# ana-kuznetsova/Policy-Gradient-ASR

Hardware: AMD Instinct MI355X
Metric: utterances/sec (B=32,T=1000,F=80) policy-grad step, 1/2/4/8 MI355X (higher is better)
Workload: dtype f32 (fp32-faithful: fp32 storage and accumulate; every big product -- recurrent sweeps, W_ih projections, input and weight gradients -- on the bf16 MFMA as SIX terms of a 3-plane split hi/mid/lo, every term down to 2^-24 of the product; the small products on the exact fp32 MFMA; the faster bf16x3 mo

## Files before the change

### include/pgasr_hip.h

```cpp
#ifndef PGASR_HIP_H
#define PGASR_HIP_H

#include <stddef.h>
#include <stdint.h>

#ifdef __cplusplus
extern "C" {
#endif

typedef enum pgasr_status {
    PGASR_OK = 0,
    PGASR_ERR_INVALID_ARG = 1,
    PGASR_ERR_LAUNCH = 2,
    PGASR_ERR_WORKSPACE = 3,
    PGASR_ERR_UNSUPPORTED = 4,
    PGASR_ERR_TIMEOUT = 5
} pgasr_status;

#define PGASR_ABI_VERSION 7

int pgasr_abi_version(void);
const char* pgasr_status_string(int status);

size_t pgasr_ctc_workspace_bytes(int T, int B, int V, int Lmax);
int pgasr_ctc_loss_grad(const float* log_probs, const int32_t* targets,
                        const int32_t* input_lengths, const int32_t* target_lengths,
                        int T, int B, int V, int Lmax, int blank,
                        const float* utt_scale, const float* pg_coef, const int32_t* pg_path,
                        float* nll, float* grad_logits,
                        void* workspace, size_t workspace_bytes, void* stream);

int pgasr_ctc_grad_from_lattice(const float* log_probs, const int32_t* input_lengths,
                                const int32_t* target_lengths, int T, int B, int V, int Lmax, int blank,
                                const float* utt_scale, const float* pg_coef, const int32_t* pg_path,
                                int pg_coef_per_frame, float* grad_logits, void* workspace, size_t workspace_bytes,
                                void* stream);

int pgasr_pg_rewards(const int32_t* dist, const int32_t* target_lengths, int B, float lam,
                     float inv_global_batch, float* R_greedy, float* R_sample, float* pg_coef,
                     float* utt_scale, void* stream);
int pgasr_pg_loss_value(const float* log_probs, const int32_t* path, const int32_t* input_lengths,
                        const float* nll, const float* utt_scale, const float* pg_coef,
                        int T, int B, int V, int pg_coef_per_frame, float* terms, void* stream);
int pgasr_pg_step_coefs(const int32_t* paths, const int32_t* input_lengths, const int32_t* prefix_dist, int prefix_stride,
                        const int32_t* token_lengths, const int32_t* target_lengths, int T, int B, int blank,
                        float lam, float inv_global_batch, float* coef, void* stream);

#define PGASR_MAX_SAMPLES 16
#define PGASR_BASELINE_HYPOTHESIS 0
#define PGASR_BASELINE_LEAVE_ONE_OUT 1
int pgasr_frame_sample_multi(const float* scores, int T, int B, int V, int K,
                             uint64_t seed, uint32_t offset, int ctr_stride, int ctr_base,
                             int32_t* greedy_path, int32_t* sample_paths, void* stream);
int pgasr_ctc_grad_from_lattice_multi(const float* log_probs, const int32_t* input_lengths,
                                      const int32_t* target_lengths, int T, int B, int V, int Lmax, int blank,
                                      const float* utt_scale, int K, const float* pg_coef, const int32_t* pg_paths,
                                      float* grad_logits, void* workspace, size_t workspace_bytes, void* stream);
int pgasr_pg_rewards_multi(const int32_t* dist, const int32_t* target_lengths, int B, int K, int baseline,
                           float lam, float inv_global_batch, float* R_baseline, float* R_sample, float* pg_coef,
                           float* utt_scale, void* stream);
int pgasr_pg_loss_value_multi(const float* log_probs, const int32_t* paths, int K, const int32_t* input_lengths,
                              const float* nll, const float* utt_scale, const float* pg_coef,
                              int T, int B, int V, float* terms, void* stream);

#define PGASR_WORD_MAX_STRIDE 4094
int pgasr_word_ids(const int32_t* ref, const int32_t* ref_len, int ref_stride,
                   const int32_t* hyp, const int32_t* hyp_len, int hyp_stride, int N, int delimiter,
                   int32_t* ref_ids, int32_t* ref_words, int32_t* hyp_ids, int32_t* hyp_words, void* stream);
int pgasr_pg_rewards_multi_ex(const int32_t* dist, const int32_t* reward_lengths, const int32_t* target_lengths, int B, int K,
                              int baseline, float lam, float inv_global_batch, float* R_baseline, float* R_sample,
                              float* pg_coef, float* utt_scale, void* stream);

int pgasr_head_logsoftmax(const float* x, long long rows, int K, int ldx, const float* W, const float* bias, int V,
                          float* logits, float* log_probs, void* stream);

int pgasr_frame_argmax_sample(const float* scores, int T, int B, int V,
                              uint64_t seed, uint32_t offset, int ctr_stride, int ctr_base,
                              int32_t* greedy_path, int32_t* sample_path, void* stream);

int pgasr_batch_prep(const float* fmask, int B, int T, const long long* tmask, const long long* targets, int L,
                     int32_t* in_len, int32_t* tg_len, int32_t* targets32, void* stream);
int pgasr_ctc_collapse(const int32_t* paths, const int32_t* lengths, int P, int T, int B,
                       int blank, int32_t* tokens, int32_t* token_lengths, void* stream);

int pgasr_edit_distance(const int32_t* ref, const int32_t* ref_len, int ref_stride,
                        const int32_t* hyp, const int32_t* hyp_len, int hyp_stride,
                        int N, int32_t* dist, int32_t* prefix_dist, void* stream);

int pgasr_reinforce_grad(const float* scores, const int32_t* path, const float* coef,
                         const int32_t* lengths, int T, int B, int V, int accumulate,
                         float* grad, void* stream);

size_t pgasr_gemm_workspace_bytes(int M, int N, int batch, int splitk, int sum_batches);
int pgasr_gemm_f32(int transA, int transB, int M, int N, int K, float alpha,
                   const float* A, int lda, long long strideA,
                   const float* B, int ldb, long long strideB,
                   float* C, int ldc, long long strideC,
                   int batch, int sum_batches, int splitk,
                   const float* bias, const float* bias2, int act, float slope, int accumulate,
                   const float* dact_y, int norm_operand, const float* shift, const float* scale,
                   int precision, const unsigned* xcc_busy, void* workspace, size_t workspace_bytes, void* stream);

int pgasr_split_bf16_planes(const float* src, int rows, int cols, int ld, int transpose,
                            unsigned short* hi, unsigned short* lo, void* stream);
int pgasr_gemm_x3w_f32(int M, int N, int K, const float* A, int lda, const unsigned short* Whi,
                       const unsigned short* Wlo, float* C, int ldc, const float* bias,
                       const float* dact_y, float slope, void* stream);
size_t pgasr_gemm_x3w_feed_workspace_bytes(void);
int pgasr_gemm_x3w_feed_col_tiles(int N);
int pgasr_gemm_x3w_feed_head_items(int N, int K, int groups);
int pgasr_gemm_x3w_feed_f32(int M, int N, int K, const float* A, int lda, const unsigned short* Whi,
                            const unsigned short* Wlo, float* C, int ldc, const float* bias,
                            const unsigned* xcc_busy, unsigned* tiles_done, int order, int phase, int head_groups,
                            void* workspace, size_t workspace_bytes, void* stream);

size_t pgasr_lstm_wgrads_workspace_bytes(int T, int in_dim);
int pgasr_lstm_wgrads_streamed(const float* dgates, const float* x, const float* out, int T, int B, int in_dim,
                               float* dwih_perm, float* dwhh_perm, const unsigned* xcc_busy,
                               const unsigned* slab_done, int* err_word, int planes,
                               void* workspace, size_t workspace_bytes, void* stream);

int pgasr_pack_x6w_planes(const float* src, int rows, int cols, int ld, int transpose, void* pack, void* stream);
int pgasr_split_bf16_planes3(const float* src, int rows, int cols, int ld, int transpose,
                             unsigned short* hi, unsigned short* mid, unsigned short* lo, void* stream);
int pgasr_gemm_x6w_f32(int M, int N, int K, const float* A, int lda, const unsigned short* Whi,
                       const unsigned short* Wmid, const unsigned short* Wlo, float* C, int ldc, const float* bias,
                       const float* dact_y, float slope, void* stream);
size_t pgasr_gemm_x6w_feed_workspace_bytes(void);
int pgasr_gemm_x6w_feed_col_tiles(int N);
int pgasr_gemm_x6w_feed_f32(int M, int N, int K, const float* A, int lda, const unsigned short* Whi,
                            const unsigned short* Wmid, const unsigned short* Wlo, float* C, int ldc, const float* bias,
                            const unsigned* xcc_busy, unsigned* tiles_done, int order,
                            void* workspace, size_t workspace_bytes, void* stream);
int pgasr_gemm_x6w_feed_head_items(int M, int N, int K);
int pgasr_gemm_x6w_feed_phase_f32(int M, int N, int K, const float* A, int lda, const unsigned short* Whi,
                                  const unsigned short* Wmid, const unsigned short* Wlo, float* C, int ldc, const float* bias,
                                  const unsigned* xcc_busy, unsigned* tiles_done, int order, int phase, unsigned* ctrl,
                                  void* workspace, size_t workspace_bytes, void* stream);

int pgasr_attention_ctx(const float* dec, const float* enc, int NQ, int B, int T, int H, float* ctx, void* stream);

int pgasr_lstm_cell_f32(const float* gh, const float* xp, float* c, float* h, float* h_out, int B, int H, void* stream);

size_t pgasr_colsum_workspace_bytes(int rows, int cols);
int pgasr_colsum_f32(const float* X, int rows, int cols, int ld, float* out, float* out2, int accumulate,
                     void* workspace, size_t workspace_bytes, void* stream);

int pgasr_instnorm_stats(const float* x, int B, int F, int T, float eps, float* mean, float* rstd,
                         void* stream);

int pgasr_log_softmax_rows(const float* logits, long long rows, int V, float* log_probs, void* stream);

size_t pgasr_lstm_pack_bytes(int which, int planes);
int pgasr_lstm_pack_weights(const float* w_ih_f, const float* w_hh_f, const float* b_ih_f, const float* b_hh_f,
                            const float* w_ih_r, const float* w_hh_r, const float* b_ih_r, const float* b_hh_r,
                            int in_dim, float* wih_perm, float* bias_perm,
                            void* whh_pack_fwd, void* whh_pack_bwd, int planes, void* stream);
int pgasr_lstm_unpack_grads(const float* dwih_perm, const float* dbias_perm, const float* dwhh_perm, int in_dim,
                            float* dw_ih_f, float* dw_hh_f, float* db_ih_f, float* db_hh_f,
                            float* dw_ih_r, float* dw_hh_r, float* db_ih_r, float* db_hh_r,
                            int accumulate, void* stream);
size_t pgasr_lstm_workspace_bytes(int T, int B, int backward);
int pgasr_lstm_error_offset(int B, int backward, size_t* offset);
int pgasr_lstm_status(const void* workspace, size_t workspace_bytes, int B, int backward, void* stream);
int pgasr_error_flag(const int32_t* word0, const int32_t* word1, float* out, void* stream);
int pgasr_lstm_busy_offset(int B, int backward, size_t* offset);
int pgasr_stream_gate(const unsigned* words, int count, int timeout_us, void* stream);
int pgasr_stream_gate_sum(const unsigned* words, int count, int need, const unsigned* running, int timeout_us, void* stream);
int pgasr_stream_gate_report(const unsigned* words, int count, int need, const unsigned* running, int timeout_us,
                             unsigned* report, void* stream);
int pgasr_stream_probe(unsigned* words, int timeout_us, void* stream);
int pgasr_lstm_layer_fwd(float* gates, float* out, float* cbuf, const void* whh_pack_fwd,
                         const int32_t* lengths, int T, int B, int flags,
                         float* out_drop, float drop_p, uint64_t drop_seed, uint32_t drop_offset,
                         void* workspace, size_t workspace_bytes, void* stream);
int pgasr_lstm_layer_fwd_fed(float* gates, float* out, float* cbuf, const void* whh_pack_fwd,
                             const int32_t* lengths, int T, int B, int flags, const unsigned* fed, int fed_need,
                             float* out_drop, float drop_p, uint64_t drop_seed, uint32_t drop_offset,
                             void* workspace, size_t workspace_bytes, void* stream);
int pgasr_lstm_fed_ok(int T, int B, int flags);
int pgasr_lstm_layer_bwd_fed(float* gates, const float* out, const float* cbuf, const float* dout,
                             const void* whh_pack_bwd, const int32_t* lengths, int T, int B, int flags,
                             float* dbias_part, const unsigned* fed, int fed_need, float drop_p, uint64_t drop_seed,
                             uint32_t drop_offset, void* workspace, size_t workspace_bytes, void* stream);
int pgasr_lstm_layer_bwd(float* gates, const float* out, const float* cbuf, const float* dout,
                         const void* whh_pack_bwd, const int32_t* lengths, int T, int B, int flags,
                         float* dbias_part, void* workspace, size_t workspace_bytes, void* stream);
int pgasr_lstm_wgrad_slabs(int T, int* edges, int max_edges);
int pgasr_lstm_layer_bwd_streamed(float* gates, const float* out, const float* cbuf, const float* dout,
                                  const void* whh_pack_bwd, const int32_t* lengths, int T, int B, int flags,
                                  float* dbias_part, const unsigned* fed, int fed_need, float drop_p, uint64_t drop_seed,
                                  uint32_t drop_offset, unsigned* slab_done,
                                  void* workspace, size_t workspace_bytes, void* stream);

size_t pgasr_beam_workspace_bytes(int T, int B, int V, int beam);
int pgasr_ctc_beam_search(const void* log_probs, int is_f64, long long stride_t, long long stride_b,
                          const int32_t* lengths, int T, int B, int V, int beam, int blank, int flags,
                          int32_t* out_tokens, int32_t* out_len, double* out_score,
                          void* workspace, size_t workspace_bytes, void* stream);

int pgasr_dropout(const float* x, float* y, unsigned long long n, float p, uint64_t seed, uint32_t offset,
                  const float* dact_y, float slope, void* stream);
int pgasr_stream_copy(const void* src, void* dst, unsigned long long bytes, int workgroups, void* stream);
int pgasr_adam_step(float* param, const float* grad, float* exp_avg, float* exp_avg_sq, unsigned long long n,
                    int step, float lr, float beta1, float beta2, float eps, float weight_decay,
                    const int32_t* guard0, const int32_t* guard1, int32_t* applied, void* stream);
#define PGASR_CLIP_STATE_BYTES 32
size_t pgasr_grad_norm_ws_bytes(unsigned long long n);
int pgasr_grad_norm_clip(const float* grad, unsigned long long n, float max_norm, void* ws, size_t ws_bytes,
                         void* state, void* stream);
int pgasr_adam_step_clipped(float* param, const float* grad, float* exp_avg, float* exp_avg_sq, unsigned long long n,
                            int step, float lr, float beta1, float beta2, float eps, float weight_decay,
                            const int32_t* guard0, const int32_t* guard1, int32_t* applied, const void* clip_state,
                            void* stream);

int pgasr_feat_frames(const float* wave, const int32_t* n_samples, const int32_t* n_frames, int B,
                      long long wave_stride, int Tmax, float* frames, void* stream);
int pgasr_feat_power(const float* spec, long long rows, float* power, void* stream);
int pgasr_feat_db(float* mel, const int32_t* n_frames, int B, int Tmax, int n_mels, float top_db, void* stream);
int pgasr_feat_deltas_stack(const float* mfcc, const int32_t* n_frames, int B, int Tmax, int n_mfcc,
                            float* feat, float* fmask, void* stream);
int pgasr_feat_stack(const float* x, const int32_t* n_frames, int B, int Tmax, int C, float* feat, float* fmask, void* stream);

#ifdef __cplusplus
}
#endif
#endif
```

### policy_gradient_asr_amd/_lib.py

```python
import ctypes as C
import os

import torch

_HERE = os.path.dirname(os.path.abspath(__file__))
LIB_PATH = os.environ.get("PGASR_HIP_LIB", os.path.join(_HERE, "libpgasr_hip.so"))

c_f32p = C.c_void_p
c_i32p = C.c_void_p
c_ptr = C.c_void_p

SIGNATURES = {
    "pgasr_abi_version": (C.c_int, []),
    "pgasr_status_string": (C.c_char_p, [C.c_int]),
    "pgasr_ctc_workspace_bytes": (C.c_size_t, [C.c_int, C.c_int, C.c_int, C.c_int]),
    "pgasr_ctc_loss_grad": (C.c_int, [c_f32p, c_i32p, c_i32p, c_i32p, C.c_int, C.c_int, C.c_int, C.c_int,
                                      C.c_int, c_f32p, c_f32p, c_i32p, c_f32p, c_f32p, c_ptr, C.c_size_t, c_ptr]),
    "pgasr_ctc_grad_from_lattice": (C.c_int, [c_f32p, c_i32p, c_i32p, C.c_int, C.c_int, C.c_int, C.c_int, C.c_int,
                                              c_f32p, c_f32p, c_i32p, C.c_int, c_f32p, c_ptr, C.c_size_t, c_ptr]),
    "pgasr_pg_rewards": (C.c_int, [c_i32p, c_i32p, C.c_int, C.c_float, C.c_float, c_f32p, c_f32p, c_f32p, c_f32p, c_ptr]),
    "pgasr_pg_loss_value": (C.c_int, [c_f32p, c_i32p, c_i32p, c_f32p, c_f32p, c_f32p, C.c_int, C.c_int, C.c_int, C.c_int,
                                      c_f32p, c_ptr]),
    "pgasr_head_logsoftmax": (C.c_int, [c_f32p, C.c_longlong, C.c_int, C.c_int, c_f32p, c_f32p, C.c_int, c_f32p, c_f32p, c_ptr]),
    "pgasr_pg_step_coefs": (C.c_int, [c_i32p, c_i32p, c_i32p, C.c_int, c_i32p, c_i32p, C.c_int, C.c_int, C.c_int,
                                      C.c_float, C.c_float, c_f32p, c_ptr]),
    "pgasr_frame_argmax_sample": (C.c_int, [c_f32p, C.c_int, C.c_int, C.c_int, C.c_uint64, C.c_uint32, C.c_int, C.c_int,
                                            c_i32p, c_i32p, c_ptr]),
    "pgasr_frame_sample_multi": (C.c_int, [c_f32p, C.c_int, C.c_int, C.c_int, C.c_int, C.c_uint64, C.c_uint32, C.c_int, C.c_int,
                                           c_i32p, c_i32p, c_ptr]),
    "pgasr_ctc_grad_from_lattice_multi": (C.c_int, [c_f32p, c_i32p, c_i32p, C.c_int, C.c_int, C.c_int, C.c_int, C.c_int,
                                                    c_f32p, C.c_int, c_f32p, c_i32p, c_f32p, c_ptr, C.c_size_t, c_ptr]),
    "pgasr_pg_rewards_multi": (C.c_int, [c_i32p, c_i32p, C.c_int, C.c_int, C.c_int, C.c_float, C.c_float, c_f32p, c_f32p, c_f32p,
                                         c_f32p, c_ptr]),
    "pgasr_pg_loss_value_multi": (C.c_int, [c_f32p, c_i32p, C.c_int, c_i32p, c_f32p, c_f32p, c_f32p, C.c_int, C.c_int, C.c_int,
                                            c_f32p, c_ptr]),
    "pgasr_word_ids": (C.c_int, [c_i32p, c_i32p, C.c_int, c_i32p, c_i32p, C.c_int, C.c_int, C.c_int, c_i32p, c_i32p, c_i32p, c_i32p,
                                 c_ptr]),
    "pgasr_pg_rewards_multi_ex": (C.c_int, [c_i32p, c_i32p, c_i32p, C.c_int, C.c_int, C.c_int, C.c_float, C.c_float, c_f32p, c_f32p,
                                            c_f32p, c_f32p, c_ptr]),
    "pgasr_batch_prep": (C.c_int, [c_f32p, C.c_int, C.c_int, c_ptr, c_ptr, C.c_int, c_i32p, c_i32p, c_i32p, c_ptr]),
    "pgasr_ctc_collapse": (C.c_int, [c_i32p, c_i32p, C.c_int, C.c_int, C.c_int, C.c_int, c_i32p, c_i32p, c_ptr]),
    "pgasr_edit_distance": (C.c_int, [c_i32p, c_i32p, C.c_int, c_i32p, c_i32p, C.c_int, C.c_int,
                                      c_i32p, c_i32p, c_ptr]),
    "pgasr_reinforce_grad": (C.c_int, [c_f32p, c_i32p, c_f32p, c_i32p, C.c_int, C.c_int, C.c_int, C.c_int,
                                       c_f32p, c_ptr]),
    "pgasr_beam_workspace_bytes": (C.c_size_t, [C.c_int] * 4),
    "pgasr_ctc_beam_search": (C.c_int, [c_ptr, C.c_int, C.c_longlong, C.c_longlong, c_i32p, C.c_int, C.c_int, C.c_int,
                                        C.c_int, C.c_int, C.c_int, c_i32p, c_i32p, c_ptr, c_ptr, C.c_size_t, c_ptr]),
    "pgasr_dropout": (C.c_int, [c_f32p, c_f32p, C.c_ulonglong, C.c_float, C.c_uint64, C.c_uint32, c_f32p, C.c_float, c_ptr]),
    "pgasr_stream_copy": (C.c_int, [c_ptr, c_ptr, C.c_ulonglong, C.c_int, c_ptr]),
    "pgasr_adam_step": (C.c_int, [c_f32p, c_f32p, c_f32p, c_f32p, C.c_ulonglong, C.c_int, C.c_float, C.c_float,
                                  C.c_float, C.c_float, C.c_float, c_i32p, c_i32p, c_i32p, c_ptr]),
    "pgasr_adam_step_clipped": (C.c_int, [c_f32p, c_f32p, c_f32p, c_f32p, C.c_ulonglong, C.c_int, C.c_float, C.c_float,
                                          C.c_float, C.c_float, C.c_float, c_i32p, c_i32p, c_i32p, c_ptr, c_ptr]),
    "pgasr_grad_norm_ws_bytes": (C.c_size_t, [C.c_ulonglong]),
    "pgasr_grad_norm_clip": (C.c_int, [c_f32p, C.c_ulonglong, C.c_float, c_ptr, C.c_size_t, c_ptr, c_ptr]),
    "pgasr_gemm_workspace_bytes": (C.c_size_t, [C.c_int] * 5),
    "pgasr_gemm_f32": (C.c_int, [C.c_int, C.c_int, C.c_int, C.c_int, C.c_int, C.c_float,
                                 c_f32p, C.c_int, C.c_longlong, c_f32p, C.c_int, C.c_longlong,
                                 c_f32p, C.c_int, C.c_longlong, C.c_int, C.c_int, C.c_int,
                                 c_f32p, c_f32p, C.c_int, C.c_float, C.c_int,
                                 c_f32p, C.c_int, c_f32p, c_f32p, C.c_int, c_ptr, c_ptr, C.c_size_t, c_ptr]),
    "pgasr_split_bf16_planes": (C.c_int, [c_f32p, C.c_int, C.c_int, C.c_int, C.c_int, c_ptr, c_ptr, c_ptr]),
    "pgasr_gemm_x3w_f32": (C.c_int, [C.c_int, C.c_int, C.c_int, c_f32p, C.c_int, c_ptr, c_ptr, c_f32p, C.c_int,
                                     c_f32p, c_f32p, C.c_float, c_ptr]),
    "pgasr_gemm_x3w_feed_workspace_bytes": (C.c_size_t, []),
    "pgasr_gemm_x3w_feed_col_tiles": (C.c_int, [C.c_int]),
    "pgasr_gemm_x3w_feed_head_items": (C.c_int, [C.c_int, C.c_int, C.c_int]),
    "pgasr_gemm_x3w_feed_f32": (C.c_int, [C.c_int, C.c_int, C.c_int, c_f32p, C.c_int, c_ptr, c_ptr, c_f32p, C.c_int,
                                          c_f32p, c_ptr, c_ptr, C.c_int, C.c_int, C.c_int, c_ptr, C.c_size_t, c_ptr]),
    "pgasr_feat_frames": (C.c_int, [c_f32p, c_i32p, c_i32p, C.c_int, C.c_longlong, C.c_int, c_f32p, c_ptr]),
    "pgasr_feat_power": (C.c_int, [c_f32p, C.c_longlong, c_f32p, c_ptr]),
    "pgasr_feat_db": (C.c_int, [c_f32p, c_i32p, C.c_int, C.c_int, C.c_int, C.c_float, c_ptr]),
    "pgasr_feat_deltas_stack": (C.c_int, [c_f32p, c_i32p, C.c_int, C.c_int, C.c_int, c_f32p, c_f32p, c_ptr]),
    "pgasr_feat_stack": (C.c_int, [c_f32p, c_i32p, C.c_int, C.c_int, C.c_int, c_f32p, c_f32p, c_ptr]),
    "pgasr_colsum_workspace_bytes": (C.c_size_t, [C.c_int, C.c_int]),
    "pgasr_colsum_f32": (C.c_int, [c_f32p, C.c_int, C.c_int, C.c_int, c_f32p, c_f32p, C.c_int,
                                   c_ptr, C.c_size_t, c_ptr]),
    "pgasr_instnorm_stats": (C.c_int, [c_f32p, C.c_int, C.c_int, C.c_int, C.c_float, c_f32p, c_f32p, c_ptr]),
    "pgasr_log_softmax_rows": (C.c_int, [c_f32p, C.c_longlong, C.c_int, c_f32p, c_ptr]),
    "pgasr_lstm_pack_bytes": (C.c_size_t, [C.c_int, C.c_int]),
    "pgasr_lstm_pack_weights": (C.c_int, [c_f32p] * 8 + [C.c_int, c_f32p, c_f32p, c_ptr, c_ptr, C.c_int, c_ptr]),
    "pgasr_lstm_unpack_grads": (C.c_int, [c_f32p, c_f32p, c_f32p, C.c_int] + [c_f32p] * 8 + [C.c_int, c_ptr]),
    "pgasr_lstm_workspace_bytes": (C.c_size_t, [C.c_int, C.c_int, C.c_int]),
    "pgasr_lstm_error_offset": (C.c_int, [C.c_int, C.c_int, C.POINTER(C.c_size_t)]),
    "pgasr_lstm_busy_offset": (C.c_int, [C.c_int, C.c_int, C.POINTER(C.c_size_t)]),
    "pgasr_lstm_status": (C.c_int, [c_ptr, C.c_size_t, C.c_int, C.c_int, c_ptr]),
    "pgasr_stream_gate": (C.c_int, [c_ptr, C.c_int, C.c_int, c_ptr]),
    "pgasr_stream_gate_sum": (C.c_int, [c_ptr, C.c_int, C.c_int, c_ptr, C.c_int, c_ptr]),
    "pgasr_stream_gate_report": (C.c_int, [c_ptr, C.c_int, C.c_int, c_ptr, C.c_int, c_ptr, c_ptr]),
    "pgasr_stream_probe": (C.c_int, [c_ptr, C.c_int, c_ptr]),
    "pgasr_lstm_layer_fwd": (C.c_int, [c_f32p, c_f32p, c_f32p, c_ptr, c_i32p, C.c_int, C.c_int, C.c_int,
                                       c_f32p, C.c_float, C.c_uint64, C.c_uint32, c_ptr, C.c_size_t, c_ptr]),
    "pgasr_lstm_layer_fwd_fed": (C.c_int, [c_f32p, c_f32p, c_f32p, c_ptr, c_i32p, C.c_int, C.c_int, C.c_int, c_ptr, C.c_int,
                                           c_f32p, C.c_float, C.c_uint64, C.c_uint32, c_ptr, C.c_size_t, c_ptr]),
    "pgasr_lstm_fed_ok": (C.c_int, [C.c_int, C.c_int, C.c_int]),
    "pgasr_lstm_layer_bwd_fed": (C.c_int, [c_f32p, c_f32p, c_f32p, c_f32p, c_ptr, c_i32p, C.c_int, C.c_int, C.c_int,
                                           c_f32p, c_ptr, C.c_int, C.c_float, C.c_uint64, C.c_uint32, c_ptr, C.c_size_t, c_ptr]),
    "pgasr_lstm_layer_bwd": (C.c_int, [c_f32p, c_f32p, c_f32p, c_f32p, c_ptr, c_i32p, C.c_int, C.c_int, C.c_int,
                                       c_f32p, c_ptr, C.c_size_t, c_ptr]),
    "pgasr_lstm_wgrad_slabs": (C.c_int, [C.c_int, c_i32p, C.c_int]),
    "pgasr_lstm_layer_bwd_streamed": (C.c_int, [c_f32p, c_f32p, c_f32p, c_f32p, c_ptr, c_i32p, C.c_int, C.c_int, C.c_int,
                                                c_f32p, c_ptr, C.c_int, C.c_float, C.c_uint64, C.c_uint32, c_ptr,
                                                c_ptr, C.c_size_t, c_ptr]),
    "pgasr_lstm_wgrads_workspace_bytes": (C.c_size_t, [C.c_int, C.c_int]),
    "pgasr_lstm_wgrads_streamed": (C.c_int, [c_f32p, c_f32p, c_f32p, C.c_int, C.c_int, C.c_int, c_f32p, c_f32p, c_ptr,
                                             c_ptr, c_ptr, C.c_int, c_ptr, C.c_size_t, c_ptr]),
    "pgasr_error_flag": (C.c_int, [c_i32p, c_i32p, c_f32p, c_ptr]),
    "pgasr_attention_ctx": (C.c_int, [c_f32p, c_f32p, C.c_int, C.c_int, C.c_int, C.c_int, c_f32p, c_ptr]),
    "pgasr_lstm_cell_f32": (C.c_int, [c_f32p, c_f32p, c_f32p, c_f32p, c_f32p, C.c_int, C.c_int, c_ptr]),
    "pgasr_pack_x6w_planes": (C.c_int, [c_f32p, C.c_int, C.c_int, C.c_int, C.c_int, c_ptr, c_ptr]),
    "pgasr_split_bf16_planes3": (C.c_int, [c_f32p, C.c_int, C.c_int, C.c_int, C.c_int, c_ptr, c_ptr, c_ptr, c_ptr]),
    "pgasr_gemm_x6w_f32": (C.c_int, [C.c_int, C.c_int, C.c_int, c_f32p, C.c_int, c_ptr, c_ptr, c_ptr, c_f32p, C.c_int,
                                     c_f32p, c_f32p, C.c_float, c_ptr]),
    "pgasr_gemm_x6w_feed_workspace_bytes": (C.c_size_t, []),
    "pgasr_gemm_x6w_feed_col_tiles": (C.c_int, [C.c_int]),
    "pgasr_gemm_x6w_feed_f32": (C.c_int, [C.c_int, C.c_int, C.c_int, c_f32p, C.c_int, c_ptr, c_ptr, c_ptr, c_f32p, C.c_int,
                                          c_f32p, c_ptr, c_ptr, C.c_int, c_ptr, C.c_size_t, c_ptr]),
    "pgasr_gemm_x6w_feed_head_items": (C.c_int, [C.c_int, C.c_int, C.c_int]),
    "pgasr_gemm_x6w_feed_phase_f32": (C.c_int, [C.c_int, C.c_int, C.c_int, c_f32p, C.c_int, c_ptr, c_ptr, c_ptr, c_f32p, C.c_int,
                                                c_f32p, c_ptr, c_ptr, C.c_int, C.c_int, c_ptr, c_ptr, C.c_size_t, c_ptr]),
}


class PgasrError(RuntimeError):
    pass


TIMEOUT = 5


_lib = None


def load():
    global _lib
    if _lib is not None:
        return _lib
    if not os.path.exists(LIB_PATH):
        raise PgasrError(
            f"{LIB_PATH} is missing: build it with `python -c 'import __graft_entry__ as g; g.build()'` "
            "or `make -C policy_gradient_asr_amd/csrc`.  There is no CPU fallback.")
    lib = C.CDLL(LIB_PATH)
    for name, (res, args) in SIGNATURES.items():
        fn = getattr(lib, name)
        fn.restype = res
        fn.argtypes = args
    if lib.pgasr_abi_version() != 7:
        raise PgasrError("libpgasr_hip.so ABI version mismatch")
    _lib = lib
    return lib


def check(status, what):
    if status != 0:
        msg = load().pgasr_status_string(status).decode()
        raise PgasrError(f"{what} failed: status {status} ({msg})")
```

### policy_gradient_asr_amd/csrc/common.h

```cpp
#pragma once
#include <hip/hip_runtime.h>
#include <stdint.h>
#include <math.h>
#include <stdio.h>
#include <stdlib.h>
#include "pgasr_hip.h"

#define PGASR_WAVE 64

#define PGASR_LAUNCH_KERNEL(...)                               \
    do {                                                       \
        (void)hipGetLastError();                               \
        hipLaunchKernelGGL(__VA_ARGS__);                       \
    } while (0)

#define PGASR_CHECK_LAUNCH()                                                                  \
    do {                                                                                      \
        hipError_t e__ = hipGetLastError();                                                   \
        if (e__ != hipSuccess) {                                                              \
            if (getenv("PGASR_DEBUG"))                                                        \
                fprintf(stderr, "[pgasr] %s:%d launch failed: %s\n", __FILE__, __LINE__,      \
                        hipGetErrorString(e__));                                              \
            return PGASR_ERR_LAUNCH;                                                          \
        }                                                                                     \
    } while (0)

static inline size_t pgasr_align_up(size_t x, size_t a) { return (x + a - 1) / a * a; }

#define PGASR_NEG_INF (-INFINITY)

__device__ __forceinline__ float wave_sum(float v) {
#pragma unroll
    for (int o = 32; o > 0; o >>= 1) v += __shfl_xor(v, o, 64);
    return v;
}
__device__ __forceinline__ float wave_max(float v) {
#pragma unroll
    for (int o = 32; o > 0; o >>= 1) v = fmaxf(v, __shfl_xor(v, o, 64));
    return v;
}

__device__ __forceinline__ void philox4x32_10(uint32_t c0, uint32_t c1, uint32_t c2, uint32_t c3,
                                              uint32_t k0, uint32_t k1, uint32_t out[4]) {
#pragma unroll
    for (int r = 0; r < 10; ++r) {
        const uint64_t p0 = (uint64_t)0xD2511F53u * c0;
        const uint64_t p1 = (uint64_t)0xCD9E8D57u * c2;
        const uint32_t n0 = (uint32_t)(p1 >> 32) ^ c1 ^ k0;
        const uint32_t n1 = (uint32_t)p1;
        const uint32_t n2 = (uint32_t)(p0 >> 32) ^ c3 ^ k1;
        const uint32_t n3 = (uint32_t)p0;
        c0 = n0; c1 = n1; c2 = n2; c3 = n3;
        k0 += 0x9E3779B9u; k1 += 0xBB67AE85u;
    }
    out[0] = c0; out[1] = c1; out[2] = c2; out[3] = c3;
}

#ifndef PGASR_WSLAB_NUM
#define PGASR_WSLAB_NUM 5
#define PGASR_WSLAB_DEN 4
#define PGASR_WSLAB_CAP 128
#endif
__host__ __device__ inline int pgasr_wslab_next(int s) { const int n = ((s * PGASR_WSLAB_NUM) / PGASR_WSLAB_DEN + 4) & ~7; return n > PGASR_WSLAB_CAP ? PGASR_WSLAB_CAP : n; }
__host__ __device__ inline int pgasr_wslab_count(int T) {
    int h = 0, s = 16, n = 1;
    while (T - h > s + s / 2) { h += s; s = pgasr_wslab_next(s); ++n; }
    return n;
}
__host__ __device__ inline int pgasr_wslab_edge(int T, int i) {
    int h = 0, s = 16;
    for (int j = 0; j < i; ++j) {
        if (T - h <= s + s / 2) return T;
        h += s; s = pgasr_wslab_next(s);
    }
    return h;
}

struct PgasrTn256Args {
    const float* A; const float* B; float* partial;
    int M, N, K, lda, ldb;
    long long sA, sB;
    int batch, splitk, kper;
    float alpha;
    unsigned* queue;
    const unsigned* xcc_busy;
    int diag;
    const unsigned* gate;
    const float* gate_base;
    int gate_T, gate_B, gate_nbg;
    int tslabs;
    int* gate_err;
};
bool pgasr_internal_tn256_ok(const PgasrTn256Args& a, int tk = 32);
int pgasr_internal_tn256_launch(PgasrTn256Args a, int masked_then_unmasked, hipStream_t st, const PgasrTn256Args* second = nullptr);
int pgasr_internal_tn6_launch(PgasrTn256Args a, int masked_then_unmasked, hipStream_t st, const PgasrTn256Args* second = nullptr);

struct PgasrX3cArgs {
    const float* A; const unsigned short* Whi; const unsigned short* Wlo; float* C;
    int M, N, K, lda, ldc;
    const float* bias; const float* dact_y; float slope;
    int feed;
    unsigned* queue; const unsigned* xcc_busy; unsigned* tiles_done;
    int mt_count, nt_count, order, quarters, split_tiles;
    float* slabs; unsigned* arrive;
};
size_t pgasr_internal_x3c_slab_bytes();
int pgasr_internal_x3c_launch(const PgasrX3cArgs& a, hipStream_t st);
```

### policy_gradient_asr_amd/csrc/gemm.hip

```cpp
#include "common.h"

namespace {

constexpr int BM = 128, BN = 128, BK = 16, PADF = 4;
constexpr int GEMM_THREADS = 256;

typedef __attribute__((ext_vector_type(16))) float f32x16;

struct GemmArgs {
    const float* A; const float* B; float* C;
    int M, N, K, lda, ldb, ldc;
    long long sA, sB, sC;
    int batch, splitk, kper;
    float alpha;
    const float* bias; const float* bias2;
    int act; float slope;
    int accumulate;
    const float* dact_y;
    int norm_operand;
    const float* shift; const float* scale;
    float* partial;
    unsigned* queue;
    const unsigned* xcc_busy;
    int tx, ty, tz;
    int wide;
};

__device__ __forceinline__ void store_tiles_fast(const GemmArgs& g, const f32x16 (&acc)[2][2], int m0, int n0, int wm, int wn,
                                                 int lane, int z, int bidx, bool live) {
    const int cl = lane & 31, rq = lane >> 5;
    if (g.partial) {
        float* slab = g.partial + (size_t)z * g.M * g.N;
        __amdgpu_buffer_rsrc_t prs = __builtin_amdgcn_make_buffer_rsrc(slab, 0, (int)(unsigned)((size_t)g.M * g.N * 4), 0x00020000);
#pragma unroll
        for (int i = 0; i < 2; ++i)
#pragma unroll
            for (int j = 0; j < 2; ++j) {
                const int n = n0 + wn * 64 + j * 32 + cl;
                const bool ok = live && n < g.N;
                const unsigned o0 = (unsigned)(((size_t)(m0 + wm * 64 + i * 32 + 4 * rq) * g.N + n) * 4);
#pragma unroll
                for (int r = 0; r < 16; ++r)
                    __builtin_amdgcn_raw_buffer_store_b32(__float_as_uint(g.alpha * acc[i][j][r]), prs,
                                                          ok ? o0 + (unsigned)(((r & 3) + 8 * (r >> 2)) * g.N * 4) : 0xFFFFFFFFu, 0, 0);
            }
        return;
    }
    float* Cb = g.C + (size_t)bidx * g.sC;
    const unsigned cbytes = (unsigned)(((size_t)(g.M - 1) * g.ldc + g.N) * 4);
    __amdgpu_buffer_rsrc_t crs = __builtin_amdgcn_make_buffer_rsrc(Cb, 0, (int)cbytes, 0x00020000);
    __amdgpu_buffer_rsrc_t yrs = __builtin_amdgcn_make_buffer_rsrc(const_cast<float*>(g.dact_y ? g.dact_y + (size_t)bidx * g.sC : Cb), 0, (int)cbytes, 0x00020000);
    float bsum[2];
#pragma unroll
    for (int j = 0; j < 2; ++j) {
        const int n = n0 + wn * 64 + j * 32 + cl;
        bsum[j] = 0.f;
        if (n < g.N) {
            if (g.bias) bsum[j] += g.bias[n];
            if (g.bias2) bsum[j] += g.bias2[n];
        }
    }
    const bool lk = g.act == 1;
    if (!g.dact_y && !g.accumulate) {
#pragma unroll
        for (int i = 0; i < 2; ++i)
#pragma unroll
            for (int j = 0; j < 2; ++j) {
                const int n = n0 + wn * 64 + j * 32 + cl;
                const bool ok = live && n < g.N;
                const unsigned o0 = (unsigned)(((size_t)(m0 + wm * 64 + i * 32 + 4 * rq) * g.ldc + n) * 4);
#pragma unroll
                for (int r = 0; r < 16; ++r) {
                    float v = g.alpha * acc[i][j][r] + bsum[j];
                    v = (lk && !(v > 0.f)) ? v * g.slope : v;
                    __builtin_amdgcn_raw_buffer_store_b32(__float_as_uint(v), crs, ok ? o0 + (unsigned)(((r & 3) + 8 * (r >> 2)) * g.ldc * 4) : 0xFFFFFFFFu, 0, 0);
                }
            }
        return;
    }
    const bool hd = g.dact_y != nullptr, ha = g.accumulate != 0;
#pragma unroll
    for (int i = 0; i < 2; ++i)
#pragma unroll
        for (int j = 0; j < 2; ++j) {
            const int n = n0 + wn * 64 + j * 32 + cl;
            const bool ok = live && n < g.N;
            const unsigned o0 = (unsigned)(((size_t)(m0 + wm * 64 + i * 32 + 4 * rq) * g.ldc + n) * 4);
            float f[16], c0[16];
#pragma unroll
            for (int r = 0; r < 16; ++r) {
                const unsigned o = ok ? o0 + (unsigned)(((r & 3) + 8 * (r >> 2)) * g.ldc * 4) : 0xFFFFFFFFu;
                f[r] = hd ? (__uint_as_float(__builtin_amdgcn_raw_buffer_load_b32(yrs, o, 0, 0)) > 0.f ? 1.f : g.slope) : 1.f;
                c0[r] = ha ? __uint_as_float(__builtin_amdgcn_raw_buffer_load_b32(crs, o, 0, 0)) : 0.f;
            }
#pragma unroll
            for (int r = 0; r < 16; ++r) {
                const unsigned o = ok ? o0 + (unsigned)(((r & 3) + 8 * (r >> 2)) * g.ldc * 4) : 0xFFFFFFFFu;
                float v = g.alpha * acc[i][j][r] + bsum[j];
                v = (lk && !(v > 0.f)) ? v * g.slope : v;
                v = v * f[r] + c0[r];
                __builtin_amdgcn_raw_buffer_store_b32(__float_as_uint(v), crs, o, 0, 0);
            }
        }
}

template <bool KCONTIG>
__device__ __forceinline__ void load_strip(const float* __restrict__ P, int ld, int mn_base, int mn_lim,
                                           int k_base, int k_lim, int tid, bool vec_ok, float v[8]) {
    if (KCONTIG) {
        const int mn = mn_base + (tid >> 1);
        const int k0 = k_base + (tid & 1) * 8;
        if (mn < mn_lim && k0 + 8 <= k_lim && vec_ok) {
            const float4* p = reinterpret_cast<const float4*>(P + (size_t)mn * ld + k0);
            const float4 a = p[0], b = p[1];
            v[0] = a.x; v[1] = a.y; v[2] = a.z; v[3] = a.w; v[4] = b.x; v[5] = b.y; v[6] = b.z; v[7] = b.w;
        } else {
#pragma unroll
            for (int i = 0; i < 8; ++i)
                v[i] = (mn < mn_lim && k0 + i < k_lim) ? P[(size_t)mn * ld + k0 + i] : 0.f;
        }
    } else {
        const int k = k_base + (tid >> 4);
        const int mn0 = mn_base + (tid & 15) * 8;
        if (k < k_lim && mn0 + 8 <= mn_lim && vec_ok) {
            const float4* p = reinterpret_cast<const float4*>(P + (size_t)k * ld + mn0);
            const float4 a = p[0], b = p[1];
            v[0] = a.x; v[1] = a.y; v[2] = a.z; v[3] = a.w; v[4] = b.x; v[5] = b.y; v[6] = b.z; v[7] = b.w;
        } else {
#pragma unroll
            for (int i = 0; i < 8; ++i)
                v[i] = (k < k_lim && mn0 + i < mn_lim) ? P[(size_t)k * ld + mn0 + i] : 0.f;
        }
    }
}

template <bool KCONTIG>
__device__ __forceinline__ void store_strip(float (*S)[BM + PADF], int tid, const float v[8]) {
    if (KCONTIG) {
        const int mn = tid >> 1, k0 = (tid & 1) * 8;
#pragma unroll
        for (int i = 0; i < 8; ++i) S[k0 + i][mn] = v[i];
    } else {
        const int k = tid >> 4, mn0 = (tid & 15) * 8;
        *reinterpret_cast<float4*>(&S[k][mn0]) = make_float4(v[0], v[1], v[2], v[3]);
        *reinterpret_cast<float4*>(&S[k][mn0 + 4]) = make_float4(v[4], v[5], v[6], v[7]);
    }
}

__device__ __forceinline__ void swizzled_tile(int& bx, int& by, int& bz) {
    const unsigned gx = gridDim.x, gy = gridDim.y, gz = gridDim.z;
    const unsigned nwg = gx * gy * gz;
    const unsigned L = blockIdx.x + gx * (blockIdx.y + gy * blockIdx.z);
    const unsigned q = nwg / 8, r = nwg % 8;
    const unsigned xcd = L % 8, i = L / 8;
    const unsigned t = (xcd < r ? xcd * (q + 1) : r * (q + 1) + (xcd - r) * q) + i;
    bx = (int)(t % gx); by = (int)((t / gx) % gy); bz = (int)(t / (gx * gy));
}

template <bool TA, bool TB>
__global__ __launch_bounds__(GEMM_THREADS) void gemm_f32_kernel(GemmArgs g) {
    __shared__ __attribute__((aligned(16))) float As[2][BK][BM + PADF];
    __shared__ __attribute__((aligned(16))) float Bs[2][BK][BN + PADF];
    const int tid = threadIdx.x, lane = tid & 63, wid = tid >> 6;
    const int wm = wid >> 1, wn = wid & 1;
    int tbx, tby, z;
    swizzled_tile(tbx, tby, z);
    const int bidx = z / g.splitk, sidx = z % g.splitk;
    const int m0 = tby * BM, n0 = tbx * BN;
    const float* A = g.A + (size_t)bidx * g.sA;
    const float* B = g.B + (size_t)bidx * g.sB;
    const int kbeg = sidx * g.kper;
    const int kend = min(g.K, kbeg + g.kper);
    const bool vecA = ((g.lda & 3) == 0) && ((((size_t)A) & 15) == 0);
    const bool vecB = ((g.ldb & 3) == 0) && ((((size_t)B) & 15) == 0);
    float nsh = 0.f, nsc = 1.f;
    if (g.norm_operand) { nsh = g.shift[bidx]; nsc = g.scale[bidx]; }

    f32x16 acc[2][2];
#pragma unroll
    for (int i = 0; i < 2; ++i)
#pragma unroll
        for (int j = 0; j < 2; ++j)
#pragma unroll
            for (int r = 0; r < 16; ++r) acc[i][j][r] = 0.f;

    float ra[8], rb[8];
    auto gload = [&](int kb) {
        load_strip<!TA>(A, g.lda, m0, g.M, kb, kend, tid, vecA, ra);
        load_strip<TB>(B, g.ldb, n0, g.N, kb, kend, tid, vecB, rb);
        if (g.norm_operand == 1) {
#pragma unroll
            for (int i = 0; i < 8; ++i) ra[i] = (ra[i] - nsh) * nsc;
        } else if (g.norm_operand == 2) {
#pragma unroll
            for (int i = 0; i < 8; ++i) rb[i] = (rb[i] - nsh) * nsc;
        }
    };
    auto fix_edges = [&](int kb) {
        if (g.norm_operand == 1) {
            if (!TA) { const int mn = m0 + (tid >> 1), k0 = kb + (tid & 1) * 8;
#pragma unroll
                for (int i = 0; i < 8; ++i) if (!(mn < g.M && k0 + i < kend)) ra[i] = 0.f; }
            else { const int k = kb + (tid >> 4), mn0 = m0 + (tid & 15) * 8;
#pragma unroll
                for (int i = 0; i < 8; ++i) if (!(k < kend && mn0 + i < g.M)) ra[i] = 0.f; }
        } else if (g.norm_operand == 2) {
            if (TB) { const int mn = n0 + (tid >> 1), k0 = kb + (tid & 1) * 8;
#pragma unroll
                for (int i = 0; i < 8; ++i) if (!(mn < g.N && k0 + i < kend)) rb[i] = 0.f; }
            else { const int k = kb + (tid >> 4), mn0 = n0 + (tid & 15) * 8;
#pragma unroll
                for (int i = 0; i < 8; ++i) if (!(k < kend && mn0 + i < g.N)) rb[i] = 0.f; }
        }
    };

    if (kbeg < kend) {
        gload(kbeg); fix_edges(kbeg);
        store_strip<!TA>(As[0], tid, ra);
        store_strip<TB>(Bs[0], tid, rb);
    }
    __syncthreads();
    int cur = 0;
    for (int kb = kbeg; kb < kend; kb += BK) {
        const bool more = kb + BK < kend;
        if (more) { gload(kb + BK); fix_edges(kb + BK); }
        const int r = lane & 31, kh = lane >> 5;
#pragma unroll
        for (int kk = 0; kk < BK; kk += 2) {
            const float a0 = As[cur][kk + kh][wm * 64 + r];
            const float a1 = As[cur][kk + kh][wm * 64 + 32 + r];
            const float b0 = Bs[cur][kk + kh][wn * 64 + r];
            const float b1 = Bs[cur][kk + kh][wn * 64 + 32 + r];
            acc[0][0] = __builtin_amdgcn_mfma_f32_32x32x2f32(a0, b0, acc[0][0], 0, 0, 0);
            acc[0][1] = __builtin_amdgcn_mfma_f32_32x32x2f32(a0, b1, acc[0][1], 0, 0, 0);
            acc[1][0] = __builtin_amdgcn_mfma_f32_32x32x2f32(a1, b0, acc[1][0], 0, 0, 0);
            acc[1][1] = __builtin_amdgcn_mfma_f32_32x32x2f32(a1, b1, acc[1][1], 0, 0, 0);
        }
        if (more) {
            store_strip<!TA>(As[cur ^ 1], tid, ra);
            store_strip<TB>(Bs[cur ^ 1], tid, rb);
        }
        __syncthreads();
        cur ^= 1;
    }

    if (!g.wide) { store_tiles_fast(g, acc, m0, n0, wm, wn, lane, z, bidx, true); return; }
    const int cl = lane & 31, rq = lane >> 5;
#pragma unroll
    for (int i = 0; i < 2; ++i)
#pragma unroll
        for (int j = 0; j < 2; ++j) {
            const int n = n0 + wn * 64 + j * 32 + cl;
            if (n >= g.N) continue;
            float bsum = 0.f;
            if (!g.partial) {
                if (g.bias) bsum += g.bias[n];
                if (g.bias2) bsum += g.bias2[n];
            }
#pragma unroll
            for (int r = 0; r < 16; ++r) {
                const int m = m0 + wm * 64 + i * 32 + (r & 3) + 8 * (r >> 2) + 4 * rq;
                if (m >= g.M) continue;
                float v = g.alpha * acc[i][j][r];
                if (g.partial) {
                    g.partial[((size_t)z * g.M + m) * g.N + n] = v;
                } else {
                    float* c = g.C + (size_t)bidx * g.sC + (size_t)m * g.ldc + n;
                    v += bsum;
                    if (g.act == 1) v = v > 0.f ? v : v * g.slope;
                    if (g.dact_y) v *= (g.dact_y[(size_t)bidx * g.sC + (size_t)m * g.ldc + n] > 0.f ? 1.f : g.slope);
                    if (g.accumulate) v += *c;
                    *c = v;
                }
            }
        }
}

constexpr int XBK = 32, XPITCH = 40;

typedef __attribute__((ext_vector_type(8))) __bf16 bf16x8_t;
typedef __attribute__((ext_vector_type(4))) unsigned u32x4_t;

__device__ __forceinline__ void split2(float x0, float x1, unsigned& hi_pk, unsigned& lo_pk) {
    typedef __attribute__((ext_vector_type(2))) __bf16 bf2;
    typedef __attribute__((ext_vector_type(2))) float f2;
    const bf2 h = __builtin_convertvector((f2){x0, x1}, bf2);
    hi_pk = __builtin_bit_cast(unsigned, h);
    const float h0 = __uint_as_float(hi_pk << 16), h1 = __uint_as_float(hi_pk & 0xFFFF0000u);
    const bf2 l = __builtin_convertvector((f2){x0 - h0, x1 - h1}, bf2);
    lo_pk = __builtin_bit_cast(unsigned, l);
}

__device__ __forceinline__ void xload_strip(const float* __restrict__ P, int ld, int mn_base, int mn_lim,
                                            int k_base, int k_lim, int tid, bool vec_ok, float v[16]) {
    const int mn = mn_base + (tid >> 1);
    const int k0 = k_base + (tid & 1) * 16;
    if (mn < mn_lim && k0 + 16 <= k_lim && vec_ok) {
        const float4* p = reinterpret_cast<const float4*>(P + (size_t)mn * ld + k0);
#pragma unroll
        for (int i = 0; i < 4; ++i) { const float4 a = p[i]; v[4 * i] = a.x; v[4 * i + 1] = a.y; v[4 * i + 2] = a.z; v[4 * i + 3] = a.w; }
    } else {
#pragma unroll
        for (int i = 0; i < 16; ++i) v[i] = (mn < mn_lim && k0 + i < k_lim) ? P[(size_t)mn * ld + k0 + i] : 0.f;
    }
}

__device__ __forceinline__ void xstore_strip(unsigned short* hi, unsigned short* lo, int tid, const float v[16]) {
    const int row = tid >> 1, k0 = (tid & 1) * 16;
    unsigned h[8], l[8];
#pragma unroll
    for (int i = 0; i < 8; ++i) split2(v[2 * i], v[2 * i + 1], h[i], l[i]);
    u32x4_t* ph = reinterpret_cast<u32x4_t*>(hi + row * XPITCH + k0);
    u32x4_t* pl = reinterpret_cast<u32x4_t*>(lo + row * XPITCH + k0);
    ph[0] = (u32x4_t){h[0], h[1], h[2], h[3]}; ph[1] = (u32x4_t){h[4], h[5], h[6], h[7]};
    pl[0] = (u32x4_t){l[0], l[1], l[2], l[3]}; pl[1] = (u32x4_t){l[4], l[5], l[6], l[7]};
}

constexpr int TPITCH = 160;
static_assert(XBK * TPITCH == BM * XPITCH, "both LDS images fill the same array");
typedef __attribute__((ext_vector_type(4))) short s16x4_t;
typedef __attribute__((ext_vector_type(8))) short s16x8_t;
typedef __attribute__((ext_vector_type(2))) unsigned u32x2_t;

__device__ __forceinline__ void tload_strip(const float* __restrict__ P, int ld, int mn_base, int mn_lim,
                                            int k_base, int k_lim, int tid, bool vec_ok, float v[16]) {
    const int mn0 = mn_base + (tid & 31) * 4;
    if (vec_ok && k_base + XBK <= k_lim && mn_base + BM <= mn_lim) {
        const float* p = P + (size_t)(k_base + (tid >> 5)) * ld + mn0;
#pragma unroll
        for (int i = 0; i < 4; ++i) {
            const float4 a = *reinterpret_cast<const float4*>(p + (size_t)(8 * i) * ld);
            v[4 * i] = a.x; v[4 * i + 1] = a.y; v[4 * i + 2] = a.z; v[4 * i + 3] = a.w;
        }
        return;
    }
#pragma unroll
    for (int i = 0; i < 4; ++i) {
        const int k = k_base + (tid >> 5) + 8 * i;
#pragma unroll
        for (int c = 0; c < 4; ++c) v[4 * i + c] = (k < k_lim && mn0 + c < mn_lim) ? P[(size_t)k * ld + mn0 + c] : 0.f;
    }
}

__device__ __forceinline__ void tstore_strip(unsigned short* hi, unsigned short* lo, int tid, const float v[16]) {
#pragma unroll
    for (int i = 0; i < 4; ++i) {
        unsigned h0, l0, h1, l1;
        split2(v[4 * i], v[4 * i + 1], h0, l0);
        split2(v[4 * i + 2], v[4 * i + 3], h1, l1);
        const int o = ((tid >> 5) + 8 * i) * TPITCH + (tid & 31) * 4;
        *reinterpret_cast<u32x2_t*>(hi + o) = (u32x2_t){h0, h1};
        *reinterpret_cast<u32x2_t*>(lo + o) = (u32x2_t){l0, l1};
    }
}

__device__ __forceinline__ bf16x8_t tr_frag(const unsigned short* p) {
    typedef s16x4_t __attribute__((address_space(3))) * lds_s16x4_ptr;
    const s16x4_t a = __builtin_amdgcn_ds_read_tr16_b64_v4i16((lds_s16x4_ptr)(p));
    const s16x4_t b = __builtin_amdgcn_ds_read_tr16_b64_v4i16((lds_s16x4_ptr)(p + 4 * TPITCH));
    return __builtin_bit_cast(bf16x8_t, (s16x8_t){a.x, a.y, a.z, a.w, b.x, b.y, b.z, b.w});
}

template <bool TA, bool TB, bool QUEUE>
__global__ __launch_bounds__(GEMM_THREADS, 2) void gemm_bf16x3_kernel(GemmArgs g) {
    __shared__ __attribute__((aligned(16))) unsigned short S[2][2][2][BM * XPITCH];
    const int tid = threadIdx.x, lane = tid & 63, wid = tid >> 6;
    const int wm = wid >> 1, wn = wid & 1;
    int tbx = 0, tby = 0, z = 0;
    bool live = true;
    if (QUEUE) {
        const unsigned xcc = __builtin_amdgcn_s_getreg(((4 - 1) << 11) | (0 << 6) | 20) & 0xFu;
        const bool allowed = g.xcc_busy == nullptr ||
                             __hip_atomic_load(g.xcc_busy + (xcc & 7u), __ATOMIC_RELAXED, __HIP_MEMORY_SCOPE_AGENT) == 0u;
        unsigned* mailbox = reinterpret_cast<unsigned*>(&S[0][0][0][0]);
        if (tid == 0) *mailbox = allowed ? __hip_atomic_fetch_add(g.queue, 1u, __ATOMIC_RELAXED, __HIP_MEMORY_SCOPE_AGENT) : 0xFFFFFFFFu;
        __syncthreads();
        const unsigned t = *mailbox;
        __syncthreads();
        live = t < (unsigned)g.tx * g.ty * g.tz;
        if (live) { tbx = (int)(t % g.tx); tby = (int)((t / g.tx) % g.ty); z = (int)(t / ((unsigned)g.tx * g.ty)); }
    } else {
        swizzled_tile(tbx, tby, z);
    }
    const int bidx = z / g.splitk, sidx = z % g.splitk;
    const int m0 = tby * BM, n0 = tbx * BN;
    const float* A = g.A + (size_t)bidx * g.sA;
    const float* B = g.B + (size_t)bidx * g.sB;
    const int kbeg = sidx * g.kper;
    const int kend = live ? min(g.K, kbeg + g.kper) : kbeg;
    const bool vecA = ((g.lda & 3) == 0) && ((((size_t)A) & 15) == 0);
    const bool vecB = ((g.ldb & 3) == 0) && ((((size_t)B) & 15) == 0);

    f32x16 acc[2][2];
#pragma unroll
    for (int i = 0; i < 2; ++i)
#pragma unroll
        for (int j = 0; j < 2; ++j)
#pragma unroll
// ... 125 lines not shown
    if (bias2) v += bias2[n];
    if (act == 1) v = v > 0.f ? v : v * slope;
    float* c = C + (size_t)m * ldc + n;
    if (accumulate) v += *c;
    *c = v;
}

__global__ __launch_bounds__(256) void colsum_partial_kernel(const float* __restrict__ X, int rows, int cols, int ld,
                                                             int rows_per_block, float* __restrict__ partial) {
    __shared__ float red[4][64];
    const int c = blockIdx.x * 64 + (threadIdx.x & 63);
    const int rl = threadIdx.x >> 6;
    const int r0 = blockIdx.y * rows_per_block, r1 = min(rows, r0 + rows_per_block);
    float s = 0.f;
    if (c < cols)
        for (int r = r0 + rl; r < r1; r += 4) s += X[(size_t)r * ld + c];
    red[rl][threadIdx.x & 63] = s;
    __syncthreads();
    if (rl == 0 && c < cols)
        partial[(size_t)blockIdx.y * cols + c] = (red[0][threadIdx.x] + red[1][threadIdx.x]) + (red[2][threadIdx.x] + red[3][threadIdx.x]);
}
__global__ __launch_bounds__(256) void colsum_final_kernel(const float* __restrict__ partial, int nparts, int cols,
                                                           float* __restrict__ out, float* __restrict__ out2, int accumulate) {
    const int c = blockIdx.x * 256 + threadIdx.x;
    if (c >= cols) return;
    float s = 0.f;
    for (int p = 0; p < nparts; ++p) s += partial[(size_t)p * cols + c];
    if (accumulate) { out[c] += s; if (out2) out2[c] += s; }
    else { out[c] = s; if (out2) out2[c] = s; }
}

__global__ __launch_bounds__(1024) void instnorm_stats_kernel(const float* __restrict__ x, long long n_per, float eps,
                                                              float* __restrict__ mean, float* __restrict__ rstd) {
    __shared__ double s1[16], s2[16];
    const float* p = x + (size_t)blockIdx.x * n_per;
    double a = 0.0, b = 0.0;
    long long done = 0;
    if (((n_per & 3) == 0) && ((((size_t)x) & 15) == 0)) {
        const float4* p4 = reinterpret_cast<const float4*>(p);
        const long long n4 = n_per >> 2;
        double a1 = 0.0, b1 = 0.0;
        long long i = threadIdx.x;
        for (; i + 3 * 1024 < n4; i += 4 * 1024) {
            const float4 u0 = p4[i], u1 = p4[i + 1024], u2 = p4[i + 2 * 1024], u3 = p4[i + 3 * 1024];
            a += ((double)u0.x + (double)u0.y) + ((double)u0.z + (double)u0.w);
            b += ((double)u0.x * u0.x + (double)u0.y * u0.y) + ((double)u0.z * u0.z + (double)u0.w * u0.w);
            a1 += ((double)u1.x + (double)u1.y) + ((double)u1.z + (double)u1.w);
            b1 += ((double)u1.x * u1.x + (double)u1.y * u1.y) + ((double)u1.z * u1.z + (double)u1.w * u1.w);
            a += ((double)u2.x + (double)u2.y) + ((double)u2.z + (double)u2.w);
            b += ((double)u2.x * u2.x + (double)u2.y * u2.y) + ((double)u2.z * u2.z + (double)u2.w * u2.w);
            a1 += ((double)u3.x + (double)u3.y) + ((double)u3.z + (double)u3.w);
            b1 += ((double)u3.x * u3.x + (double)u3.y * u3.y) + ((double)u3.z * u3.z + (double)u3.w * u3.w);
        }
        for (; i < n4; i += 1024) {
            const float4 u = p4[i];
            a += ((double)u.x + (double)u.y) + ((double)u.z + (double)u.w);
            b += ((double)u.x * u.x + (double)u.y * u.y) + ((double)u.z * u.z + (double)u.w * u.w);
        }
        a += a1; b += b1;
        done = n_per;
    }
    for (long long i = done + threadIdx.x; i < n_per; i += 1024) { const double v = p[i]; a += v; b += v * v; }
#pragma unroll
    for (int o = 32; o > 0; o >>= 1) { a += __shfl_xor(a, o, 64); b += __shfl_xor(b, o, 64); }
    if ((threadIdx.x & 63) == 0) { s1[threadIdx.x >> 6] = a; s2[threadIdx.x >> 6] = b; }
    __syncthreads();
    if (threadIdx.x == 0) {
        double ta = 0.0, tb = 0.0;
        for (int i = 0; i < 16; ++i) { ta += s1[i]; tb += s2[i]; }
        const double mu = ta / (double)n_per;
        double var = tb / (double)n_per - mu * mu;
        if (var < 0.0) var = 0.0;
        mean[blockIdx.x] = (float)mu;
        rstd[blockIdx.x] = (float)(1.0 / sqrt(var + (double)eps));
    }
}

}

static int gemm_launch(GemmArgs& g, int transA, int transB, int sum_batches, int precision, const unsigned* xcc_busy, void* workspace,
                       size_t workspace_bytes, hipStream_t st) {
    const int Z = g.batch * g.splitk;
    const bool use_partial = (g.splitk > 1) || sum_batches;
    const bool queue_mode = precision >= 1 && xcc_busy != nullptr;
    const size_t head = 256;
    if (use_partial || queue_mode) {
        const size_t need = head + (use_partial ? (size_t)Z * g.M * g.N * sizeof(float) : 0);
        if (!workspace || workspace_bytes < need) return PGASR_ERR_WORKSPACE;
    }
    g.partial = use_partial ? (float*)((char*)workspace + head) : nullptr;
    g.queue = nullptr; g.xcc_busy = nullptr;
    dim3 grid((g.N + BN - 1) / BN, (g.M + BM - 1) / BM, Z);
    if (grid.y > 65535 || grid.z > 65535) return PGASR_ERR_UNSUPPORTED;
    g.tx = (int)grid.x; g.ty = (int)grid.y; g.tz = (int)grid.z;
    if (queue_mode) {
        g.queue = (unsigned*)workspace; g.xcc_busy = xcc_busy;
        if (hipMemsetAsync(workspace, 0, head, st) != hipSuccess) return PGASR_ERR_LAUNCH;
    }
    const unsigned ntiles_q = grid.x * grid.y * grid.z;

    bool done_tn256 = false;
    if (precision >= 1 && transA && !transB && use_partial && g.norm_operand == 0) {
        PgasrTn256Args t{g.A, g.B, g.partial, g.M, g.N, g.K, g.lda, g.ldb, g.sA, g.sB, g.batch, g.splitk, g.kper, g.alpha,
                         queue_mode ? g.queue : nullptr, queue_mode ? g.xcc_busy : nullptr, getenv("PGASR_TN_DIAG") ? atoi(getenv("PGASR_TN_DIAG")) : 0,
                         nullptr, nullptr, 0, 0, 0, 0, nullptr};
        if (pgasr_internal_tn256_ok(t)) {
            const int st_ = precision == 2 ? pgasr_internal_tn6_launch(t, queue_mode ? 1 : 0, st) : pgasr_internal_tn256_launch(t, queue_mode ? 1 : 0, st);
            if (st_ != PGASR_OK) return st_;
            done_tn256 = true;
        }
    }
    if (done_tn256) {
    }
    else if (precision == 2) return PGASR_ERR_UNSUPPORTED;
    else if (precision == 1) {
        if (queue_mode) {
            for (int pass = 0; pass < 2; ++pass) {
                dim3 qgrid(pass == 0 ? 2u * ntiles_q + 8u : ntiles_q);
                if (pass == 1) g.xcc_busy = nullptr;
                if (!transA && !transB) PGASR_LAUNCH_KERNEL((gemm_bf16x3_kernel<false, false, true>), qgrid, dim3(GEMM_THREADS), 0, st, g);
                else if (!transA && transB) PGASR_LAUNCH_KERNEL((gemm_bf16x3_kernel<false, true, true>), qgrid, dim3(GEMM_THREADS), 0, st, g);
                else if (transA && !transB) PGASR_LAUNCH_KERNEL((gemm_bf16x3_kernel<true, false, true>), qgrid, dim3(GEMM_THREADS), 0, st, g);
                else PGASR_LAUNCH_KERNEL((gemm_bf16x3_kernel<true, true, true>), qgrid, dim3(GEMM_THREADS), 0, st, g);
                PGASR_CHECK_LAUNCH();
            }
        }
        else if (!transA && !transB) PGASR_LAUNCH_KERNEL((gemm_bf16x3_kernel<false, false, false>), grid, dim3(GEMM_THREADS), 0, st, g);
        else if (!transA && transB) PGASR_LAUNCH_KERNEL((gemm_bf16x3_kernel<false, true, false>), grid, dim3(GEMM_THREADS), 0, st, g);
        else if (transA && !transB) PGASR_LAUNCH_KERNEL((gemm_bf16x3_kernel<true, false, false>), grid, dim3(GEMM_THREADS), 0, st, g);
        else PGASR_LAUNCH_KERNEL((gemm_bf16x3_kernel<true, true, false>), grid, dim3(GEMM_THREADS), 0, st, g);
    }
    else if (!transA && !transB) PGASR_LAUNCH_KERNEL((gemm_f32_kernel<false, false>), grid, dim3(GEMM_THREADS), 0, st, g);
    else if (!transA && transB) PGASR_LAUNCH_KERNEL((gemm_f32_kernel<false, true>), grid, dim3(GEMM_THREADS), 0, st, g);
    else if (transA && !transB) PGASR_LAUNCH_KERNEL((gemm_f32_kernel<true, false>), grid, dim3(GEMM_THREADS), 0, st, g);
    else PGASR_LAUNCH_KERNEL((gemm_f32_kernel<true, true>), grid, dim3(GEMM_THREADS), 0, st, g);
    PGASR_CHECK_LAUNCH();
    if (use_partial) {
        const size_t total = (size_t)g.M * g.N;
        const int nout = sum_batches ? 1 : g.batch;
        PGASR_LAUNCH_KERNEL(gemm_reduce_kernel, dim3((unsigned)((total + 255) / 256), nout), dim3(256), 0, st,
                           g.partial, Z / nout, g.M, g.N, g.C, g.ldc, g.sC, g.bias, g.bias2, g.act, g.slope,
                           g.accumulate);
        PGASR_CHECK_LAUNCH();
    }
    return PGASR_OK;
}

extern "C" size_t pgasr_gemm_workspace_bytes(int M, int N, int batch, int splitk, int sum_batches) {
    if (M <= 0 || N <= 0 || batch <= 0 || splitk <= 0) return 0;
    if (splitk <= 1 && !sum_batches) return 256;
    return 256 + (size_t)batch * splitk * M * N * sizeof(float);
}

extern "C" int pgasr_gemm_f32(int transA, int transB, int M, int N, int K, float alpha,
                              const float* A, int lda, long long strideA,
                              const float* B, int ldb, long long strideB,
                              float* C, int ldc, long long strideC,
                              int batch, int sum_batches, int splitk,
                              const float* bias, const float* bias2, int act, float slope, int accumulate,
                              const float* dact_y, int norm_operand, const float* shift, const float* scale,
                              int precision, const unsigned* xcc_busy, void* workspace, size_t workspace_bytes, void* stream) {
    if (!A || !B || !C || M <= 0 || N <= 0 || K <= 0 || batch <= 0 || splitk <= 0) return PGASR_ERR_INVALID_ARG;
    if (norm_operand < 0 || norm_operand > 2 || (norm_operand && (!shift || !scale))) return PGASR_ERR_INVALID_ARG;
    if (act < 0 || act > 1 || precision < 0 || precision > 2) return PGASR_ERR_INVALID_ARG;
    if ((splitk > 1 || sum_batches) && dact_y) return PGASR_ERR_INVALID_ARG;
    GemmArgs g;
    g.A = A; g.B = B; g.C = C; g.M = M; g.N = N; g.K = K; g.lda = lda; g.ldb = ldb; g.ldc = ldc;
    g.sA = strideA; g.sB = strideB; g.sC = strideC; g.batch = batch; g.splitk = splitk;
    int kper = (K + splitk - 1) / splitk;
    const int kq = precision >= 1 ? XBK : BK;
    kper = (kper + kq - 1) / kq * kq;
    g.kper = kper;
    g.alpha = alpha; g.bias = bias; g.bias2 = bias2; g.act = act; g.slope = slope; g.accumulate = accumulate;
    g.dact_y = dact_y; g.norm_operand = norm_operand; g.shift = shift; g.scale = scale; g.partial = nullptr;
    g.wide = (((size_t)(M - 1) * ldc + N) * 4 >= ((size_t)1 << 32) || (size_t)M * N * 4 >= ((size_t)1 << 32)) ? 1 : 0;
    return gemm_launch(g, transA, transB, sum_batches, precision, xcc_busy, workspace, workspace_bytes, (hipStream_t)stream);
}

extern "C" int pgasr_lstm_wgrad_slabs(int T, int* edges, int max_edges) {
    if (T <= 0) return 0;
    const int n = pgasr_wslab_count(T);
    for (int i = 0; edges && i <= n && i < max_edges; ++i) edges[i] = pgasr_wslab_edge(T, i);
    return n;
}
extern "C" size_t pgasr_lstm_wgrads_workspace_bytes(int T, int in_dim) {
    if (in_dim <= 0 || T <= 0) return 0;
    return 256 + (size_t)pgasr_wslab_count(T) * ((size_t)2048 * in_dim + (size_t)2 * 1024 * 256) * sizeof(float);
}
extern "C" int pgasr_lstm_wgrads_streamed(const float* dgates, const float* x, const float* out, int T, int B, int in_dim,
                                          float* dwih_perm, float* dwhh_perm, const unsigned* xcc_busy,
                                          const unsigned* slab_done, int* err_word, int planes,
                                          void* workspace, size_t workspace_bytes, void* stream) {
    constexpr int H = 256, G = 2 * 4 * H;
    if (!dgates || !x || !out || !dwih_perm || !dwhh_perm || T <= 1 || B <= 0 || in_dim <= 0) return PGASR_ERR_INVALID_ARG;
    if (planes != 2 && planes != 3) return PGASR_ERR_INVALID_ARG;
    const size_t need = pgasr_lstm_wgrads_workspace_bytes(T, in_dim);
    if (!workspace || workspace_bytes < need) return PGASR_ERR_WORKSPACE;
    hipStream_t st = (hipStream_t)stream;
    const int nslab = pgasr_wslab_count(T);
    float* part_ih = (float*)((char*)workspace + 256);
    float* part_hh = part_ih + (size_t)nslab * G * in_dim;
    const long long K_ih = (long long)T * B, K_hh = (long long)(T - 1) * B;
    if (K_ih >= ((long long)1 << 31)) return PGASR_ERR_UNSUPPORTED;
    PgasrTn256Args ih{dgates, x, part_ih, G, in_dim, (int)K_ih, G, in_dim, 0, 0, 1, nslab, 0, 1.f,
                      (unsigned*)workspace, xcc_busy, 0, slab_done, dgates, T, B, (B + 15) / 16, 1, err_word};
    PgasrTn256Args hh{dgates + (size_t)B * G, out, part_hh, 4 * H, H, (int)K_hh, G, 2 * H, (long long)4 * H - (long long)B * G,
                      (long long)B * 2 * H + H, 2, nslab, 0, 1.f,
                      (unsigned*)workspace, xcc_busy, 0, slab_done, dgates, T, B, (B + 15) / 16, 1, err_word};
    const int tk = planes == 3 ? 16 : 32;
    if (!pgasr_internal_tn256_ok(ih, tk) || !pgasr_internal_tn256_ok(hh, tk)) return PGASR_ERR_UNSUPPORTED;
    if (hipMemsetAsync(workspace, 0, 256, st) != hipSuccess) return PGASR_ERR_LAUNCH;
    const int rc = planes == 3 ? pgasr_internal_tn6_launch(ih, 1, st, &hh) : pgasr_internal_tn256_launch(ih, 1, st, &hh);
    if (rc != PGASR_OK) return rc;
    PGASR_LAUNCH_KERNEL(gemm_reduce_kernel, dim3((unsigned)(((size_t)G * in_dim + 255) / 256), 1), dim3(256), 0, st,
                       part_ih, nslab, G, in_dim, dwih_perm, in_dim, (long long)0, (const float*)nullptr, (const float*)nullptr, 0, 0.f, 0);
    PGASR_CHECK_LAUNCH();
    PGASR_LAUNCH_KERNEL(gemm_reduce_kernel, dim3((unsigned)(((size_t)4 * H * H + 255) / 256), 2), dim3(256), 0, st,
                       part_hh, nslab, 4 * H, H, dwhh_perm, H, (long long)4 * H * H, (const float*)nullptr, (const float*)nullptr, 0, 0.f, 0);
    PGASR_CHECK_LAUNCH();
    return PGASR_OK;
}

extern "C" size_t pgasr_colsum_workspace_bytes(int rows, int cols) {
    if (rows <= 0 || cols <= 0) return 0;
    const int rpb = 512;
    return (size_t)((rows + rpb - 1) / rpb) * cols * sizeof(float);
}

extern "C" int pgasr_colsum_f32(const float* X, int rows, int cols, int ld, float* out, float* out2, int accumulate,
                                void* workspace, size_t workspace_bytes, void* stream) {
    if (!X || !out || rows <= 0 || cols <= 0 || ld < cols) return PGASR_ERR_INVALID_ARG;
    const int rpb = 512;
    const int nparts = (rows + rpb - 1) / rpb;
    if (!workspace || workspace_bytes < (size_t)nparts * cols * sizeof(float)) return PGASR_ERR_WORKSPACE;
    hipStream_t st = (hipStream_t)stream;
    PGASR_LAUNCH_KERNEL(colsum_partial_kernel, dim3((cols + 63) / 64, nparts), dim3(256), 0, st, X, rows, cols, ld, rpb,
                       (float*)workspace);
    PGASR_CHECK_LAUNCH();
    PGASR_LAUNCH_KERNEL(colsum_final_kernel, dim3((cols + 255) / 256), dim3(256), 0, st, (const float*)workspace, nparts,
                       cols, out, out2, accumulate);
    PGASR_CHECK_LAUNCH();
    return PGASR_OK;
}

extern "C" int pgasr_instnorm_stats(const float* x, int B, int F, int T, float eps, float* mean, float* rstd,
                                    void* stream) {
    if (!x || !mean || !rstd || B <= 0 || F <= 0 || T <= 0) return PGASR_ERR_INVALID_ARG;
    PGASR_LAUNCH_KERNEL(instnorm_stats_kernel, dim3(B), dim3(1024), 0, (hipStream_t)stream, x, (long long)F * T, eps,
                       mean, rstd);
    PGASR_CHECK_LAUNCH();
    return PGASR_OK;
}
```

### policy_gradient_asr_amd/csrc/optim.hip

```cpp
#include "common.h"

namespace {

__device__ __forceinline__ void keep4(unsigned long long quad, uint32_t offset, uint32_t k0, uint32_t k1,
                                      uint32_t thresh, bool keep[4]) {
    uint32_t r[4];
    philox4x32_10((uint32_t)quad, (uint32_t)(quad >> 32), offset, 0u, k0, k1, r);
#pragma unroll
    for (int i = 0; i < 4; ++i) keep[i] = r[i] >= thresh;
}

__global__ __launch_bounds__(256) void dropout_kernel(const float* __restrict__ x, float* __restrict__ y,
                                                      unsigned long long n, uint32_t thresh, float scale,
                                                      uint32_t k0, uint32_t k1, uint32_t offset,
                                                      const float* __restrict__ dact_y, float slope) {
    const unsigned long long nq = (n + 3) / 4;
    for (unsigned long long q = (unsigned long long)blockIdx.x * 256 + threadIdx.x; q < nq;
         q += (unsigned long long)gridDim.x * 256) {
        bool keep[4];
        keep4(q, offset, k0, k1, thresh, keep);
        const unsigned long long i = q * 4;
        if (i + 4 <= n) {
            float4 v = *reinterpret_cast<const float4*>(x + i);
            if (dact_y) {
                const float4 a = *reinterpret_cast<const float4*>(dact_y + i);
                v.x *= a.x > 0.f ? 1.f : slope; v.y *= a.y > 0.f ? 1.f : slope;
                v.z *= a.z > 0.f ? 1.f : slope; v.w *= a.w > 0.f ? 1.f : slope;
            }
            float4 o;
            o.x = keep[0] ? v.x * scale : 0.f; o.y = keep[1] ? v.y * scale : 0.f;
            o.z = keep[2] ? v.z * scale : 0.f; o.w = keep[3] ? v.w * scale : 0.f;
            *reinterpret_cast<float4*>(y + i) = o;
        } else {
            for (int k = 0; k < 4 && i + k < n; ++k)
                y[i + k] = keep[k] ? x[i + k] * scale * (dact_y ? (dact_y[i + k] > 0.f ? 1.f : slope) : 1.f) : 0.f;
        }
    }
}

struct ClipState { float norm, scale; int32_t nonfinite, pad, n_clipped, n_nonfinite, pad2[2]; };

template <bool CLIP>
__global__ __launch_bounds__(256) void adam_kernel(float* __restrict__ p, const float* __restrict__ g,
                                                   float* __restrict__ m, float* __restrict__ v, unsigned long long n,
                                                   float lr, float beta1, float beta2, float eps, int call,
                                                   float weight_decay, const int32_t* __restrict__ guard0,
                                                   const int32_t* __restrict__ guard1, int32_t* __restrict__ applied,
                                                   const ClipState* __restrict__ clip) {
    bool skip = (guard0 && *guard0 != 0) || (guard1 && *guard1 != 0);
    float gscale = 1.f;
    if (CLIP) {
        skip = skip || clip->nonfinite != 0;
        gscale = clip->scale;
    }
    int eff = call;
    if (applied) {
        const int before = applied[(call - 1) & 1];
        eff = before + 1;
        if (blockIdx.x == 0 && threadIdx.x == 0) applied[call & 1] = skip ? before : eff;
    }
    if (skip) return;
    const float bc1 = 1.f - powf(beta1, (float)eff);
    const float bc2_sqrt = sqrtf(1.f - powf(beta2, (float)eff));
    const float step = lr / bc1;
    for (unsigned long long i = ((unsigned long long)blockIdx.x * 256 + threadIdx.x) * 4; i < n;
         i += (unsigned long long)gridDim.x * 256 * 4) {
        if (i + 4 <= n) {
            float4 pp = *reinterpret_cast<float4*>(p + i);
            const float4 gg = *reinterpret_cast<const float4*>(g + i);
            float4 mm = *reinterpret_cast<float4*>(m + i);
            float4 vv = *reinterpret_cast<float4*>(v + i);
            float* P = &pp.x; const float* G = &gg.x; float* M = &mm.x; float* V = &vv.x;
#pragma unroll
            for (int k = 0; k < 4; ++k) {
                const float gk = (CLIP ? __fmul_rn(gscale, G[k]) : G[k]) + weight_decay * P[k];
                M[k] = beta1 * M[k] + (1.f - beta1) * gk;
                V[k] = beta2 * V[k] + (1.f - beta2) * gk * gk;
                P[k] -= step * M[k] / (sqrtf(V[k]) / bc2_sqrt + eps);
            }
            *reinterpret_cast<float4*>(p + i) = pp;
            *reinterpret_cast<float4*>(m + i) = mm;
            *reinterpret_cast<float4*>(v + i) = vv;
        } else {
            for (unsigned long long k = i; k < n; ++k) {
                const float gk = (CLIP ? __fmul_rn(gscale, g[k]) : g[k]) + weight_decay * p[k];
                m[k] = beta1 * m[k] + (1.f - beta1) * gk;
                v[k] = beta2 * v[k] + (1.f - beta2) * gk * gk;
                p[k] -= step * m[k] / (sqrtf(v[k]) / bc2_sqrt + eps);
            }
        }
    }
}

#define PGASR_NORM_MAX_BLOCKS 1024
__host__ __device__ inline unsigned grad_norm_blocks(unsigned long long n) {
    const unsigned long long b = ((n + 3) / 4 + 255) / 256;
    return b > PGASR_NORM_MAX_BLOCKS ? PGASR_NORM_MAX_BLOCKS : (unsigned)b;
}

__device__ __forceinline__ double wave_sum_f64(double v) {
#pragma unroll
    for (int o = 32; o > 0; o >>= 1) {
        const int lo = __shfl_xor(__double2loint(v), o, 64), hi = __shfl_xor(__double2hiint(v), o, 64);
        v += __hiloint2double(hi, lo);
    }
    return v;
}

__device__ __forceinline__ double sumsq4(double acc, const float4 q) {
    acc += (double)q.x * (double)q.x; acc += (double)q.y * (double)q.y;
    acc += (double)q.z * (double)q.z; acc += (double)q.w * (double)q.w;
    return acc;
}

__global__ __launch_bounds__(256) void grad_norm_partial_kernel(const float* __restrict__ g, unsigned long long n,
                                                                double* __restrict__ partial) {
    const unsigned long long nq = n / 4;
    const unsigned long long stride = (unsigned long long)gridDim.x * 256;
    const float4* __restrict__ g4 = reinterpret_cast<const float4*>(g);
    unsigned long long q = (unsigned long long)blockIdx.x * 256 + threadIdx.x;
    double acc = 0.0;
    for (; q + 3 * stride < nq; q += 4 * stride) {
        const float4 a = g4[q], b = g4[q + stride], c = g4[q + 2 * stride], d = g4[q + 3 * stride];
        acc = sumsq4(sumsq4(sumsq4(sumsq4(acc, a), b), c), d);
    }
    for (; q < nq; q += stride) acc = sumsq4(acc, g4[q]);
    if (blockIdx.x == 0 && threadIdx.x == 0)
        for (unsigned long long k = nq * 4; k < n; ++k) acc += (double)g[k] * (double)g[k];
    __shared__ double wsum[4];
    acc = wave_sum_f64(acc);
    if ((threadIdx.x & 63) == 0) wsum[threadIdx.x >> 6] = acc;
    __syncthreads();
    if (threadIdx.x == 0) partial[blockIdx.x] = ((wsum[0] + wsum[1]) + wsum[2]) + wsum[3];
}

__global__ __launch_bounds__(64) void grad_norm_final_kernel(const double* __restrict__ partial, unsigned blocks, float max_norm,
                                                             ClipState* __restrict__ st) {
    double part[PGASR_NORM_MAX_BLOCKS / 64];
#pragma unroll
    for (int k = 0; k < PGASR_NORM_MAX_BLOCKS / 64; ++k) {
        const unsigned i = threadIdx.x + 64u * k;
        part[k] = i < blocks ? partial[i] : 0.0;
    }
    double acc = 0.0;
#pragma unroll
    for (int k = 0; k < PGASR_NORM_MAX_BLOCKS / 64; ++k) acc += part[k];
    acc = wave_sum_f64(acc);
    if (threadIdx.x == 0) {
        const float norm = (float)sqrt(acc);
        const bool bad = !(acc < INFINITY);
        const float scale = bad ? 0.f : fminf(1.f, __fdiv_rn(max_norm, norm + 1e-6f));
        st->norm = norm;
        st->scale = scale;
        st->nonfinite = bad ? 1 : 0;
        if (bad) st->n_nonfinite += 1;
        else if (scale < 1.f) st->n_clipped += 1;
    }
}

typedef unsigned v4u __attribute__((ext_vector_type(4)));
__global__ __launch_bounds__(256) void stream_copy_kernel(const v4u* __restrict__ src, v4u* __restrict__ dst,
                                                          unsigned long long n16, const unsigned char* __restrict__ src_tail,
                                                          unsigned char* __restrict__ dst_tail, unsigned tail) {
// ... 115 lines not shown
```

### policy_gradient_asr_amd/functional.py

```python
import os

import torch

from . import hipops
from . import streams

HID = hipops.HID
FEED_AHEAD = os.environ.get("PGASR_FEED_AHEAD", "1") != "0"
JOIN_FEED = os.environ.get("PGASR_JOIN_FEED", "0") == "1"
FEED_BWD = os.environ.get("PGASR_FEED_BWD", "1") != "0"
STREAM_DW = os.environ.get("PGASR_STREAM_DW", "1") != "0"
LEAKY_SLOPE = 0.01


def _pick_splitk(M, N, K, target_wgs=512, batch=1, beside_sweep=False):
    if M % 256 == 0 and N % 256 == 0 and K % 32 == 0 and K >= 64:
        tiles = (M // 256) * (N // 256) * batch
        sk = max(1, min((128 if beside_sweep else 256) // tiles, K // 256))
        while sk > 1 and (sk - 1) * (-(-K // sk // 32) * 32) >= K:
            sk -= 1
        return sk
    tiles = ((M + 127) // 128) * ((N + 127) // 128)
    sk = max(1, min(64, target_wgs // max(tiles, 1)))
    while sk > 1 and K // sk < 256:
        sk //= 2
    return max(sk, 1)


class grad_overlap:
    enabled = False
    confine = os.environ.get("PGASR_CONFINE", "1") != "0"
    confine_feed = os.environ.get("PGASR_CONFINE_FEED", "1") != "0"
    _sides = {}
    _pendings = {}

    @classmethod
    def _key(cls):
        return torch.cuda.current_stream().cuda_stream

    _main_of = {}

    @classmethod
    def side_stream(cls):
        k = cls._key()
        if k not in cls._sides:
            cls._sides[k] = streams.side_stream("weight_gradients")
            cls._main_of[cls._sides[k].cuda_stream] = k
        return cls._sides[k]

    upper_grads_hook = None
    tail_dx_first = os.environ.get("PGASR_TAIL_DX_FIRST", "1") != "0"
    split_tail = True
    _sides2 = {}

    @classmethod
    def second_side_stream(cls):
        k = cls._key()
        if k not in cls._sides2:
            cls._sides2[k] = streams.side_stream("feed")
        return cls._sides2[k]

    _sides3 = {}
    _streamed_unjoined = {}

    @classmethod
    def third_side_stream(cls):
        k = cls._key()
        if k not in cls._sides3:
            cls._sides3[k] = streams.side_stream("streamed_weight_gradients")
        return cls._sides3[k]

    _recent = {}
    _feed_unjoined = {}

    @classmethod
    def note_event(cls, ev):
        cls._recent[cls._key()] = ev

    @classmethod
    def take_event(cls):
        return cls._recent.pop(cls._key(), None)

    @classmethod
    def pending(cls):
        return cls._pendings.setdefault(cls._key(), [])

    _deferred = {}

    @classmethod
    def flush(cls, busy_ptr=0, launched_after=None, first=None):
        pending = cls.pending()
        if not pending and first is None:
            return
        side = cls.side_stream()
        prev = hipops.GEMM_XCC_BUSY_PTR
        hipops.GEMM_XCC_BUSY_PTR = busy_ptr if cls.confine else 0
        try:
            with torch.cuda.stream(side):
                for ready, fn in pending:
                    side.wait_event(ready)
                if launched_after is not None and busy_ptr:
                    side.wait_event(launched_after)
                    hipops.stream_gate(busy_ptr)
                if first is not None:
                    first()
                for ready, fn in pending:
                    fn()
        finally:
            hipops.GEMM_XCC_BUSY_PTR = prev
            del pending[:]

    @classmethod
    def finish(cls):
        if cls._deferred:
            cls._deferred.clear()
            raise RuntimeError("a deferred input gradient was never consumed by a BLSTM layer (grad_overlap/FEED_AHEAD)")
        cls.flush()
        cls._recent.pop(cls._key(), None)
        if cls._key() in cls._sides:
            torch.cuda.current_stream().wait_stream(cls.side_stream())
        if cls._streamed_unjoined.pop(cls._key(), False) and cls._key() in cls._sides3:
            torch.cuda.current_stream().wait_stream(cls._sides3[cls._key()])
        if cls._feed_unjoined.pop(cls._key(), False) and cls._key() in cls._sides2:
            torch.cuda.current_stream().wait_stream(cls.second_side_stream())


AFFINE_DW_SPLITK = 2


class InstNormAffineFn(torch.autograd.Function):

    @staticmethod
    def forward(ctx, x, weight, bias, consumer_applies_dact=False):
        B, F, T = x.shape
        N = weight.shape[0]
        x = x.contiguous(); weight = weight.contiguous(); bias = bias.contiguous()
        ctx.consumer_applies_dact = bool(consumer_applies_dact)
        mean, rstd = hipops.instnorm_stats(x, 1e-5)
        y = torch.empty(T, B, N, dtype=torch.float32, device=x.device)
        hipops.gemm(x, weight, y, M=T, N=N, K=F, transA=True, transB=True, lda=T, ldb=F, ldc=B * N,
                    strideA=F * T, strideB=0, strideC=N, batch=B, bias=bias, act=1, slope=LEAKY_SLOPE,
                    norm_operand=1, shift=mean, scale=rstd, precision=0)
        ctx.save_for_backward(x, weight, mean, rstd, y)
        ctx.bias_ref, ctx.weight_ref = bias, weight
        return y

    @staticmethod
    def backward(ctx, dy):
        x, weight, mean, rstd, y = ctx.saved_tensors
        B, F, T = x.shape
        N = weight.shape[0]
        if ctx.consumer_applies_dact:
            dpre = dy.contiguous()
        else:
            dpre = torch.where(y > 0, dy, dy * LEAKY_SLOPE).contiguous()
        bg = getattr(ctx.bias_ref, "grad", None)
        if grad_overlap.enabled and bg is not None and bg.is_contiguous() and bg.dtype == torch.float32:
            main = torch.cuda.current_stream()
            side = grad_overlap.side_stream()
            ready = torch.cuda.Event()
            ready.record()
            with torch.cuda.stream(side):
                side.wait_event(ready)
                hipops.colsum(dpre, T * B, N, N, bg, accumulate=True)
            streams.hold(dpre, side)
            wg = getattr(ctx.weight_ref, "grad", None)
            direct = wg is not None and wg.is_contiguous() and wg.dtype == torch.float32 and tuple(wg.shape) == (N, F)
            dW = wg if direct else torch.empty(N, F, dtype=torch.float32, device=x.device)
            hipops.gemm(dpre, x, dW, M=N, N=F, K=T, transA=True, transB=True, lda=B * N, ldb=T, ldc=F,
                        strideA=N, strideB=F * T, strideC=0, batch=B, sum_batches=True, norm_operand=2,
                        shift=mean, scale=rstd, accumulate=direct, splitk=AFFINE_DW_SPLITK if T >= 256 else 1)
            return (None, None if direct else dW, None, None)
        return (None, *InstNormAffineFn.param_grads(x, mean, rstd, dpre, N), None)

    @staticmethod
    def param_grads(x, mean, rstd, dpre, N):
        B, F, T = x.shape
        dW = torch.empty(N, F, dtype=torch.float32, device=x.device)
        hipops.gemm(dpre, x, dW, M=N, N=F, K=T, transA=True, transB=True, lda=B * N, ldb=T, ldc=F,
                    strideA=N, strideB=F * T, strideC=0, batch=B, sum_batches=True, norm_operand=2,
                    shift=mean, scale=rstd, splitk=AFFINE_DW_SPLITK if T >= 256 else 1)
        db = torch.empty(N, dtype=torch.float32, device=x.device)
        hipops.colsum(dpre, T * B, N, N, db)
        return dW, db


class DropoutFn(torch.autograd.Function):

    @staticmethod
    def forward(ctx, x, p, seed, offset, *opt):
        ctx.cfg = (float(p), int(seed), int(offset))
        x = x.contiguous()
        ctx.fused = bool(opt[0]) if opt else False
        ctx.nopt = len(opt)
        if ctx.fused:
            ctx.save_for_backward(x)
        return hipops.dropout(x, p, seed, offset)

    @staticmethod
    def backward(ctx, dy):
        p, seed, offset = ctx.cfg
        rec = grad_overlap._deferred.get(dy.data_ptr())
        if rec is not None and not ctx.fused and rec["drop"] is None and dy.shape == rec["dx"].shape:
            rec["drop"] = (p, seed, offset)
            return (dy, None, None, None) + (None,) * ctx.nopt
        dact = ctx.saved_tensors[0] if ctx.fused else None
        return (hipops.dropout(dy.contiguous(), p, seed, offset, dact_y=dact, slope=LEAKY_SLOPE), None, None, None) + (None,) * ctx.nopt


class LinearFn(torch.autograd.Function):

    @staticmethod
    def forward(ctx, x, weight, bias):
        shp = x.shape
        x2 = x.contiguous().view(-1, shp[-1])
        rows, K = x2.shape
        N = weight.shape[0]
        weight = weight.contiguous()
        y = torch.empty(rows, N, dtype=torch.float32, device=x.device)
        hipops.gemm(x2, weight, y, M=rows, N=N, K=K, transB=True, bias=bias.contiguous())
        ctx.save_for_backward(x2, weight)
        ctx.shp = shp
        ctx.param_refs = (weight, bias)
        return y.view(*shp[:-1], N)

    @staticmethod
    def backward(ctx, dy):
        x2, weight = ctx.saved_tensors
        rows, K = x2.shape
        N = weight.shape[0]
        dy2 = dy.contiguous().view(rows, N)
        dx = torch.empty(rows, K, dtype=torch.float32, device=dy.device)
        hipops.gemm(dy2, weight, dx, M=rows, N=K, K=N)
        wg, bg = (p.grad for p in ctx.param_refs)
        if grad_overlap.enabled and wg is not None and bg is not None and wg.is_contiguous() and bg.is_contiguous():
            done = torch.cuda.Event()
            done.record()
            grad_overlap.note_event(done)

            def weight_grads():
                hipops.gemm(dy2, x2, wg, M=N, N=K, K=rows, transA=True, lda=N, splitk=_pick_splitk(N, K, rows), accumulate=True)
                hipops.colsum(dy2, rows, N, N, bg, accumulate=True)
            grad_overlap.pending().append((done, weight_grads))
            side = grad_overlap.side_stream()
            streams.hold(dy2, side); streams.hold(x2, side)
            return dx.view(ctx.shp), None, None
        dW = torch.empty(N, K, dtype=torch.float32, device=dy.device)
        hipops.gemm(dy2, x2, dW, M=N, N=K, K=rows, transA=True, lda=N, splitk=_pick_splitk(N, K, rows))
        db = torch.empty(N, dtype=torch.float32, device=dy.device)
        hipops.colsum(dy2, rows, N, N, db)
        return dx.view(ctx.shp), dW, db


class HeadFn(torch.autograd.Function):

    @staticmethod
    def forward(ctx, x, weight, bias):
        shp = x.shape
        x2 = x.contiguous().view(-1, shp[-1])
        weight = weight.contiguous()
        logits, lp = hipops.head_logsoftmax(x2, weight, bias.contiguous())
        ctx.save_for_backward(x2, weight)
        ctx.shp = shp
        ctx.param_refs = (weight, bias)
        lp = lp.view(*shp[:-1], -1)
        ctx.mark_non_differentiable(lp)
        return logits.view(*shp[:-1], -1), lp

    @staticmethod
    def backward(ctx, dy, _dlp=None):
        return LinearFn.backward(ctx, dy)


class LogSoftmaxFn(torch.autograd.Function):
    @staticmethod
    def forward(ctx, logits):
        lp = hipops.log_softmax_rows(logits.contiguous())
        ctx.save_for_backward(lp)
        return lp

    @staticmethod
    def backward(ctx, g):
        (lp,) = ctx.saved_tensors
        return g - torch.exp(lp) * g.sum(dim=-1, keepdim=True)


class BLSTMLayerFn(torch.autograd.Function):

    @staticmethod
    def forward(ctx, x, lengths, dact_y, sweep_follows, prepacked, out_dropout, w_ih_f, w_hh_f, b_ih_f, b_hh_f, w_ih_r, w_hh_r, b_ih_r, b_hh_r):
        T, B, I = x.shape
        x = x.contiguous()
        if prepacked is None:
            prepacked = prepack_blstm((w_ih_f, w_hh_f, b_ih_f, b_hh_f, w_ih_r, w_hh_r, b_ih_r, b_hh_r), I)
        elif prepacked.ready is not None:
            torch.cuda.current_stream().wait_event(prepacked.ready)
        wih_perm, bias_perm, pack_f, pack_b = prepacked.wih_perm, prepacked.bias_perm, prepacked.pack_f, prepacked.pack_b
        ctx.planes_t = prepacked.planes_t
        npl = len(prepacked.planes) if prepacked.planes is not None else hipops.LSTM_PLANES
        ctx.nplanes = npl
        ctx.fed_bwd = prepacked.fed_bwd
        prepacked.fed_bwd = None
        ctx.slab_words = prepacked.slab
        prepacked.slab = None
        G = 2 * 4 * HID
        gates = torch.empty(T, B, G, dtype=torch.float32, device=x.device)
        out = torch.empty(T, B, 2 * HID, dtype=torch.float32, device=x.device)
        cbuf = torch.empty(T, B, 2 * HID, dtype=torch.float32, device=x.device)
        ctx.out_dropout = tuple(out_dropout) if out_dropout is not None else None
        out_drop = torch.empty_like(out) if out_dropout is not None else None
        dkw = {"out_drop": out_drop, "drop": ctx.out_dropout}
        x3w = prepacked.planes is not None and hipops.gemm_x3w_ok(T * B, G, I, planes=npl)
        if (x3w and FEED_AHEAD and hipops.lstm_fed_ok(T, B) and hipops.x3w_feed_col_tiles(G, npl) > 0
                and hipops.streams_concurrent(grad_overlap.second_side_stream())):
            main = torch.cuda.current_stream()
            side = grad_overlap.second_side_stream()
            need_words = 2 * ((T * B + 255) // 256)
            done = prepacked.fed_fwd if (prepacked.fed_fwd is not None and prepacked.fed_fwd.numel() >= need_words) else None
            prepacked.fed_fwd = None
            if done is None:
                done = torch.zeros(need_words, dtype=torch.int32, device=x.device)
            head = hipops.x3w_feed_head_items(G, I, planes=npl) > 0
            ws_feed = hipops.gemm_x3w_feed(x, prepacked.planes, gates, T * B, G, I, bias_perm, 0, done, phase=1) if head else None
            zeroed = torch.cuda.Event()
            zeroed.record()
            hipops.lstm_layer_fwd(gates, out, cbuf, pack_f, lengths, T, B, fed=done, fed_need=hipops.x3w_feed_col_tiles(G, npl), **dkw)
            side.wait_event(zeroed)
            busy = hipops.lstm_busy_ptr(T, B, False, x.device)
            with torch.cuda.stream(side):
                hipops.stream_gate(busy)
                hipops.gemm_x3w_feed(x, prepacked.planes, gates, T * B, G, I, bias_perm, busy if grad_overlap.confine_feed else 0, done,
                                     phase=2 if head else 0, ws=ws_feed)
            if ws_feed is not None:
                streams.hold(ws_feed, side)
            for t_ in (x, gates, done, bias_perm) + tuple(prepacked.planes):
                streams.hold(t_, side)
            grad_overlap._feed_unjoined[main.cuda_stream] = True
            if JOIN_FEED:
                main.wait_stream(side)
        else:
            if x3w and npl == 3 and hipops.x3w_feed_col_tiles(G, npl) > 0 and T * B * G * 4 < 2 ** 31:
                hipops.gemm_x3w_feed(x, prepacked.planes, gates, T * B, G, I, bias_perm, 0,
                                     torch.zeros(2 * ((T * B + 255) // 256), dtype=torch.int32, device=x.device))
            elif x3w:
                hipops.gemm_x3w(x, prepacked.planes, gates, T * B, G, I, bias=bias_perm)
            else:
                hipops.gemm(x, wih_perm, gates, M=T * B, N=G, K=I, transB=True, bias=bias_perm)
            hipops.lstm_layer_fwd(gates, out, cbuf, pack_f, lengths, T, B, **dkw)
        ctx.save_for_backward(x, lengths, gates, out, cbuf, wih_perm, pack_b, dact_y if dact_y is not None else x.new_empty(0))
        ctx.has_dact = dact_y is not None
        ctx.sweep_follows = bool(sweep_follows)
        ctx.param_refs = (w_ih_f, w_hh_f, b_ih_f, b_hh_f, w_ih_r, w_hh_r, b_ih_r, b_hh_r)
        return out if out_drop is None else out_drop

    @staticmethod
    def backward(ctx, dout):
        x, lengths, gates, out, cbuf, wih_perm, pack_b, dact_y = ctx.saved_tensors
        T, B, I = x.shape
        G = 2 * 4 * HID
        dev = x.device
        npl = ctx.nplanes
        dout = dout.contiguous()
        rec = grad_overlap._deferred.pop(dout.data_ptr(), None) if grad_overlap.enabled else None
        if ctx.out_dropout is not None:
            if rec is not None and rec["drop"] is None and dout.shape == rec["dx"].shape:
                rec["drop"] = ctx.out_dropout
            else:
                dout = hipops.dropout(dout, *ctx.out_dropout)
        if grad_overlap.enabled:
            before = grad_overlap.take_event()
            if before is None:
                before = torch.cuda.Event()
                before.record()
        targets = [p.grad for p in ctx.param_refs]
        stream_own = (grad_overlap.enabled and STREAM_DW and all(t is not None and t.is_contiguous() for t in targets)
                      and hipops.lstm_wgrads_ok(T, B, I, npl) and hipops.lstm_fed_ok(T, B)
                      and hipops.streams_concurrent(grad_overlap.third_side_stream()))
        slab = None
        if stream_own:
            slab = ctx.slab_words if (ctx.slab_words is not None and ctx.slab_words.numel() >= 64) else None
            ctx.slab_words = None
            if slab is None:
                slab = torch.zeros(64, dtype=torch.int32, device=dev)
        if rec is not None:
            if grad_overlap.enabled and rec["head"]():
                before = torch.cuda.Event()
                before.record()
            sweep_ws, dbias_part = hipops.lstm_layer_bwd(gates, out, cbuf, dout, pack_b, lengths, T, B, want_dbias=True,
                                                         fed=rec["done"], fed_need=rec["need"], drop=rec["drop"], slab=slab)
        else:
            sweep_ws, dbias_part = hipops.lstm_layer_bwd(gates, out, cbuf, dout, pack_b, lengths, T, B, want_dbias=True, slab=slab)
        dg = gates
        if grad_overlap.enabled:
            busy = hipops.lstm_busy_ptr(T, B, True, dev)
            grad_overlap.flush(busy, launched_after=before, first=(lambda: rec["launch"](busy)) if rec is not None else None)
            if rec is not None:
                streams.hold(dout, grad_overlap.side_stream())
            fed_done = None
            if stream_own and grad_overlap._key() in grad_overlap._sides:
                fed_done = torch.cuda.Event()
                with torch.cuda.stream(grad_overlap.side_stream()):
                    fed_done.record()
# ... 183 lines not shown
```

### policy_gradient_asr_amd/hipops.py

```python
import os

import torch

_os_environ_get = os.environ.get

from . import _lib


def _stream():
    return torch.cuda.current_stream().cuda_stream


def _req(t, dtype, name):
    if t is None:
        return None
    if not t.is_cuda:
        raise _lib.PgasrError(f"{name} must live on the GPU (got {t.device}); there is no CPU path")
    if t.dtype != dtype:
        raise _lib.PgasrError(f"{name} must be {dtype} (got {t.dtype})")
    if not t.is_contiguous():
        raise _lib.PgasrError(f"{name} must be contiguous")
    return t


# ... 268 lines not shown
    _req(scores, torch.float32, "scores")
    T, B, V = scores.shape
    g = torch.empty(T, B, dtype=torch.int32, device=scores.device) if want_greedy else None
    s = torch.empty(T, B, dtype=torch.int32, device=scores.device) if want_sample else None
    st = lib.pgasr_frame_argmax_sample(_p(scores), T, B, V, int(seed) & (2 ** 64 - 1), int(offset) & 0xFFFFFFFF,
                                       int(batch_stride), int(batch_offset), _p(g), _p(s), _stream())
    _lib.check(st, "pgasr_frame_argmax_sample")
    return g, s


def frame_sample_multi(scores, num_samples, seed=0, offset=0, want_greedy=False, batch_stride=0, batch_offset=0, out=None):
    lib = _lib.load()
    _req(scores, torch.float32, "scores")
    T, B, V = scores.shape
    K = int(num_samples)
    if out is not None:
        g, s = out
        _req(g, torch.int32, "out greedy"); _req(s, torch.int32, "out samples")
        if tuple(s.shape) != (K, T, B) or (g is not None and tuple(g.shape) != (T, B)):
            raise _lib.PgasrError(f"frame_sample_multi: out tensors must be ({T},{B}) and ({K},{T},{B}) int32")
    else:
        g = torch.empty(T, B, dtype=torch.int32, device=scores.device) if want_greedy else None
        s = torch.empty(K, T, B, dtype=torch.int32, device=scores.device)
    st = lib.pgasr_frame_sample_multi(_p(scores), T, B, V, K, int(seed) & (2 ** 64 - 1), int(offset) & 0xFFFFFFFF,
                                      int(batch_stride), int(batch_offset), _p(g), _p(s), _stream())
    _lib.check(st, "pgasr_frame_sample_multi")
    return g, s


def batch_prep(fmask, tmask, targets):
    lib = _lib.load()
    _req(fmask, torch.float32, "fmask"); _req(tmask, torch.int64, "tmask"); _req(targets, torch.int64, "targets")
    B, T = fmask.shape
    L = targets.shape[1]
    if tuple(tmask.shape) != (B, L) or targets.shape[0] != B:
        raise _lib.PgasrError("batch_prep: fmask (B,T), tmask (B,L), targets (B,L)")
    dev = fmask.device
    in_len = torch.empty(B, dtype=torch.int32, device=dev)
    tg_len = torch.empty(B, dtype=torch.int32, device=dev)
    tg32 = torch.empty(B, L, dtype=torch.int32, device=dev)
    _lib.check(lib.pgasr_batch_prep(_p(fmask), B, T, _p(tmask), _p(targets), L, _p(in_len), _p(tg_len), _p(tg32), _stream()), "pgasr_batch_prep")
    return in_len, tg_len, tg32


def ctc_collapse(paths, lengths, blank=0, out=None):
    lib = _lib.load()
    _req(paths, torch.int32, "paths"); _req(lengths, torch.int32, "lengths")
    P, T, B = paths.shape
    if out is not None:
        tokens, tl = out
        _req(tokens, torch.int32, "out tokens"); _req(tl, torch.int32, "out lengths")
        if tokens.numel() != P * B * T or tl.numel() != P * B:
            raise _lib.PgasrError("ctc_collapse: out tensors must hold (P,B,T) and (P,B) int32")
    else:
        tokens = torch.zeros(P, B, T, dtype=torch.int32, device=paths.device)
        tl = torch.empty(P, B, dtype=torch.int32, device=paths.device)
    st = lib.pgasr_ctc_collapse(_p(paths), _p(lengths), P, T, B, blank, _p(tokens), _p(tl), _stream())
    _lib.check(st, "pgasr_ctc_collapse")
    return tokens, tl


def edit_distance(ref, ref_len, hyp, hyp_len, want_prefix=False):
    lib = _lib.load()
    _req(ref, torch.int32, "ref"); _req(hyp, torch.int32, "hyp")
    _req(ref_len, torch.int32, "ref_len"); _req(hyp_len, torch.int32, "hyp_len")
    N, R = ref.shape
    Hy = hyp.shape[1]
    dist = torch.empty(N, dtype=torch.int32, device=ref.device)
    prefix = torch.full((N, Hy + 1), -1, dtype=torch.int32, device=ref.device) if want_prefix else None
    st = lib.pgasr_edit_distance(_p(ref) if R else 0, _p(ref_len), R, _p(hyp) if Hy else 0, _p(hyp_len), Hy,
                                 N, _p(dist), _p(prefix), _stream())
    _lib.check(st, "pgasr_edit_distance")
    return (dist, prefix) if want_prefix else dist


WORD_MAX_STRIDE = 4094


def word_ids(ref, ref_len, hyp, hyp_len, delimiter):
    lib = _lib.load()
    _req(ref, torch.int32, "ref"); _req(hyp, torch.int32, "hyp")
    _req(ref_len, torch.int32, "ref_len"); _req(hyp_len, torch.int32, "hyp_len")
    N, R = ref.shape
    Hy = hyp.shape[1]
    dev = ref.device
    ref_ids = torch.empty(N, R + 1, dtype=torch.int32, device=dev)
    hyp_ids = torch.empty(N, Hy + 1, dtype=torch.int32, device=dev)
    counts = torch.empty(2, N, dtype=torch.int32, device=dev)
    st = lib.pgasr_word_ids(_p(ref) if R else 0, _p(ref_len), R, _p(hyp) if Hy else 0, _p(hyp_len), Hy, N, int(delimiter),
                            _p(ref_ids), counts[0].data_ptr(), _p(hyp_ids), counts[1].data_ptr(), _stream())
    _lib.check(st, "pgasr_word_ids")
    return ref_ids, counts[0], hyp_ids, counts[1]


def word_edit_distance(ref, ref_len, hyp, hyp_len, delimiter):
    ref_ids, ref_words, hyp_ids, hyp_words = word_ids(ref, ref_len, hyp, hyp_len, delimiter)
    return edit_distance(ref_ids, ref_words, hyp_ids, hyp_words), ref_words, hyp_words


def reinforce_grad(scores, path, coef, lengths, out=None, accumulate=False):
    lib = _lib.load()
    _req(scores, torch.float32, "scores"); _req(path, torch.int32, "path")
    _req(coef, torch.float32, "coef"); _req(lengths, torch.int32, "lengths")
    T, B, V = scores.shape
    if out is None:
        if accumulate:
            raise _lib.PgasrError("accumulate=True needs an output tensor")
        out = torch.empty_like(scores)
    _req(out, torch.float32, "out")
    st = lib.pgasr_reinforce_grad(_p(scores), _p(path), _p(coef), _p(lengths), T, B, V, int(bool(accumulate)),
                                  _p(out), _stream())
    _lib.check(st, "pgasr_reinforce_grad")
    return out


GEMM_XCC_BUSY_PTR = 0
GEMM_PRECISION = 0
LSTM_PLANES = 3

PRECISION_MODES = {"bf16x3": (1, 2), "f32": (0, 3)}
_precision = "f32"


def set_precision(mode):
    global GEMM_PRECISION, LSTM_PLANES, _precision
    if mode not in PRECISION_MODES:
        raise ValueError(f"precision mode must be one of {sorted(PRECISION_MODES)}")
    GEMM_PRECISION, LSTM_PLANES = PRECISION_MODES[mode]
    _precision = mode


def get_precision():
    return _precision


class precision:

    def __init__(self, mode):
        self.mode = mode

    def __enter__(self):
        self.prev = _precision
        set_precision(self.mode)
        return self

    def __exit__(self, *a):
        set_precision(self.prev)
        return False


def gemm(A, B, C, M, N, K, transA=False, transB=False, lda=None, ldb=None, ldc=None, alpha=1.0,
         strideA=0, strideB=0, strideC=0, batch=1, sum_batches=False, splitk=1, bias=None, bias2=None,
         act=0, slope=0.01, accumulate=False, dact_y=None, norm_operand=0, shift=None, scale=None,
         a_off=0, b_off=0, c_off=0, precision=None, xcc_busy=None):
    lib = _lib.load()
    if precision is None:
        precision = GEMM_PRECISION
    for t, nm in ((A, "A"), (B, "B"), (C, "C"), (bias, "bias"), (bias2, "bias2"), (dact_y, "dact_y"),
                  (shift, "shift"), (scale, "scale")):
        if t is not None:
            if not t.is_cuda or t.dtype != torch.float32:
                raise _lib.PgasrError(f"gemm operand {nm} must be a float32 GPU tensor")
    lda = lda if lda is not None else (M if transA else K)
    ldb = ldb if ldb is not None else (K if transB else N)
    ldc = ldc if ldc is not None else N
    nbytes = lib.pgasr_gemm_workspace_bytes(M, N, batch, splitk, int(sum_batches))
    ws = _workspace(nbytes, C.device, "gemm")
    with _timed("gemm_f32"):
      st = lib.pgasr_gemm_f32(int(transA), int(transB), M, N, K, float(alpha),
                            A.data_ptr() + 4 * a_off, lda, int(strideA), B.data_ptr() + 4 * b_off, ldb, int(strideB),
                            C.data_ptr() + 4 * c_off, ldc, int(strideC), batch, int(sum_batches), splitk,
                            _p(bias), _p(bias2), act, float(slope), int(accumulate), _p(dact_y),
                            norm_operand, _p(shift), _p(scale), int(precision), int(GEMM_XCC_BUSY_PTR if xcc_busy is None else xcc_busy), _p(ws), ws.numel() if ws is not None else 0, _stream())
    _lib.check(st, "pgasr_gemm_f32")
    return C


X6_PACKED = _os_environ_get("PGASR_X6_PACKED", "1") != "0"


class X6Pack:
    __slots__ = ("pack", "N", "K")

    def __init__(self, pack, N, K):
        self.pack, self.N, self.K = pack, N, K

    def __len__(self):
        return 3

    def __iter__(self):
        return iter((self.pack,))


def split_planes(w, transpose=False, planes=None, packed=None):
    lib = _lib.load()
    _req(w, torch.float32, "w")
    if w.dim() != 2 or w.stride(1) != 1:
        raise _lib.PgasrError("split_planes wants a row-major 2-D tensor")
    planes = LSTM_PLANES if planes is None else int(planes)
    if planes not in (2, 3):
        raise _lib.PgasrError("split_planes: 2 or 3 planes")
    rows, cols = w.shape
    shape = (cols, rows) if transpose else (rows, cols)
    if planes == 3 and (X6_PACKED if packed is None else packed) and shape[0] % 256 == 0 and shape[1] % 16 == 0:
        pack = torch.empty(shape[0] * shape[1] * 6, dtype=torch.uint8, device=w.device)
        _lib.check(lib.pgasr_pack_x6w_planes(w.data_ptr(), rows, cols, w.stride(0), int(transpose), pack.data_ptr(), _stream()), "pgasr_pack_x6w_planes")
        return X6Pack(pack, shape[0], shape[1])
    out = tuple(torch.empty(shape, dtype=torch.int16, device=w.device) for _ in range(planes))
    if planes == 3:
        st = lib.pgasr_split_bf16_planes3(w.data_ptr(), rows, cols, w.stride(0), int(transpose), *[t.data_ptr() for t in out], _stream())
    else:
        st = lib.pgasr_split_bf16_planes(w.data_ptr(), rows, cols, w.stride(0), int(transpose), *[t.data_ptr() for t in out], _stream())
    _lib.check(st, "pgasr_split_bf16_planes")
    return out


def gemm_x3w_ok(M, N, K, lda=None, planes=2):
    lda = K if lda is None else lda
    if planes == 3:
        Mp = (M + 255) // 256 * 256
        return K % 16 == 0 and K >= 64 and N % 256 == 0 and lda % 4 == 0 and M > 0 and Mp * max(N, lda) * 4 < 2 ** 32
    return K % 32 == 0 and N % 128 == 0 and lda % 4 == 0 and M > 0


def _plane_ptrs(planes):
    if isinstance(planes, X6Pack):
        return planes.pack.data_ptr(), None, None
    return tuple(t.data_ptr() for t in planes)


def _check_planes(planes, N, K, what):
    if isinstance(planes, X6Pack):
        if (planes.N, planes.K) != (N, K) or not planes.pack.is_cuda:
            raise _lib.PgasrError(f"{what}: packed planes are for a ({planes.N}, {planes.K}) weight, the product wants ({N}, {K})")
        return
    if len(planes) not in (2, 3):
        raise _lib.PgasrError(f"{what}: planes must be a (hi, lo) or (hi, mid, lo) tuple")
    for t in planes:
        if tuple(t.shape) != (N, K) or t.dtype != torch.int16 or not t.is_contiguous() or not t.is_cuda:
            raise _lib.PgasrError(f"{what} planes must be contiguous int16 (N, K) GPU tensors")


def gemm_x3w(A, planes, C, M, N, K, lda=None, ldc=None, bias=None, dact_y=None, slope=0.01):
    lib = _lib.load()
    for t, nm in ((A, "A"), (C, "C"), (bias, "bias"), (dact_y, "dact_y")):
        if t is not None and (not t.is_cuda or t.dtype != torch.float32):
            raise _lib.PgasrError(f"gemm_x3w operand {nm} must be a float32 GPU tensor")
    _check_planes(planes, N, K, "gemm_x3w")
    with _timed("gemm_x6c" if len(planes) == 3 else "gemm_x3c"):
        if len(planes) == 3:
            st = lib.pgasr_gemm_x6w_f32(M, N, K, A.data_ptr(), K if lda is None else lda, *_plane_ptrs(planes),
                                        C.data_ptr(), N if ldc is None else ldc, _p(bias), _p(dact_y), float(slope), _stream())
        else:
            st = lib.pgasr_gemm_x3w_f32(M, N, K, A.data_ptr(), K if lda is None else lda, planes[0].data_ptr(), planes[1].data_ptr(),
                                        C.data_ptr(), N if ldc is None else ldc, _p(bias), _p(dact_y), float(slope), _stream())
    _lib.check(st, "pgasr_gemm_x6w_f32" if len(planes) == 3 else "pgasr_gemm_x3w_f32")
    return C


def colsum(X, rows, cols, ld, out, out2=None, accumulate=False):
    lib = _lib.load()
    nbytes = lib.pgasr_colsum_workspace_bytes(rows, cols)
    ws = _workspace(nbytes, X.device, "colsum")
    st = lib.pgasr_colsum_f32(_p(X), rows, cols, ld, _p(out), _p(out2), int(accumulate), _p(ws), ws.numel(), _stream())
    _lib.check(st, "pgasr_colsum_f32")
    return out


def instnorm_stats(x, eps=1e-5):
    lib = _lib.load()
    _req(x, torch.float32, "x")
    B, F, T = x.shape
    mean = torch.empty(B, dtype=torch.float32, device=x.device)
    rstd = torch.empty(B, dtype=torch.float32, device=x.device)
    _lib.check(lib.pgasr_instnorm_stats(_p(x), B, F, T, float(eps), _p(mean), _p(rstd), _stream()), "pgasr_instnorm_stats")
    return mean, rstd


def log_softmax_rows(logits):
    lib = _lib.load()
    _req(logits, torch.float32, "logits")
    V = logits.shape[-1]
    out = torch.empty_like(logits)
    _lib.check(lib.pgasr_log_softmax_rows(_p(logits), logits.numel() // V, V, _p(out), _stream()), "pgasr_log_softmax_rows")
    return out


HID = 256


def lstm_pack(params, in_dim):
    lib = _lib.load()
    dev = params[0].device
    for t in params:
        _req(t, torch.float32, "lstm parameter")
    wih_perm = torch.empty(2 * 4 * HID, in_dim, dtype=torch.float32, device=dev)
    bias_perm = torch.empty(2 * 4 * HID, dtype=torch.float32, device=dev)
    nb = lib.pgasr_lstm_pack_bytes(0, LSTM_PLANES)
    pack_f = torch.empty(nb, dtype=torch.uint8, device=dev)
    pack_b = torch.empty(nb, dtype=torch.uint8, device=dev)
    st = lib.pgasr_lstm_pack_weights(*[_p(t) for t in params], in_dim, _p(wih_perm), _p(bias_perm),
                                     _p(pack_f), _p(pack_b), LSTM_PLANES, _stream())
    _lib.check(st, "pgasr_lstm_pack_weights")
    return wih_perm, bias_perm, pack_f, pack_b


def _lstm_flags(pack):
    planes = 3 if pack.numel() == _lib.load().pgasr_lstm_pack_bytes(0, 3) else 2
    return LSTM_FLAGS | (2 if planes == 3 else 0)


def lstm_unpack_grads(dwih_perm, dbias_perm, dwhh_perm, in_dim, grads, accumulate=False):
    lib = _lib.load()
    st = lib.pgasr_lstm_unpack_grads(_p(dwih_perm), _p(dbias_perm), _p(dwhh_perm), in_dim,
                                     *[_p(g) for g in grads], int(accumulate), _stream())
    _lib.check(st, "pgasr_lstm_unpack_grads")


_lstm_err_checks = []


def _lstm_ws(T, B, backward, device):
    lib = _lib.load()
    nbytes = lib.pgasr_lstm_workspace_bytes(T, B, int(backward))
    return _workspace(nbytes, device, "lstm_bwd" if backward else "lstm_fwd")


import os as _os
LSTM_FLAGS = int(_os.environ.get("PGASR_LSTM_FLAGS", "0"), 0)


def lstm_layer_fwd(gates, out, cbuf, pack_f, lengths, T, B, fed=None, fed_need=0, out_drop=None, drop=None):
    lib = _lib.load()
    ws = _lstm_ws(T, B, False, gates.device)
    p, seed, offset = drop if (drop is not None and out_drop is not None) else (0.0, 0, 0)
    if out_drop is not None:
        _req(out_drop, torch.float32, "out_drop")
        if out_drop.numel() != out.numel() or drop is None:
            raise _lib.PgasrError("lstm_layer_fwd: out_drop must have out's size and come with drop = (p, seed, offset)")
    dargs = (_p(out_drop), float(p), int(seed) & (2 ** 64 - 1), int(offset) & 0xFFFFFFFF)
    with _timed("lstm_fwd_kernel"):
        if fed is None:
            st = lib.pgasr_lstm_layer_fwd(_p(gates), _p(out), _p(cbuf), _p(pack_f), _p(lengths), T, B, _lstm_flags(pack_f), *dargs,
                                          _p(ws), ws.numel(), _stream())
        else:
            if fed.dtype != torch.int32 or not fed.is_cuda or fed.numel() < 2 * ((T * B + 255) // 256):
                raise _lib.PgasrError("lstm_layer_fwd: fed must be an int32 GPU tensor of 2 * ceil(T*B/256) words")
            st = lib.pgasr_lstm_layer_fwd_fed(_p(gates), _p(out), _p(cbuf), _p(pack_f), _p(lengths), T, B, _lstm_flags(pack_f),
                                              _p(fed), int(fed_need), *dargs, _p(ws), ws.numel(), _stream())
    _lib.check(st, "pgasr_lstm_layer_fwd_fed" if fed is not None else "pgasr_lstm_layer_fwd")
    return ws


def lstm_fed_ok(T, B):
    return bool(_lib.load().pgasr_lstm_fed_ok(T, B, LSTM_FLAGS))


def x3w_feed_col_tiles(N, planes=2):
    lib = _lib.load()
    return int(lib.pgasr_gemm_x6w_feed_col_tiles(int(N)) if planes == 3 else lib.pgasr_gemm_x3w_feed_col_tiles(int(N)))


FEED_HEAD_GROUPS = int(_os_environ_get("PGASR_FEED_HEAD", "0"))




def x3w_feed_head_items(N, K, groups=None, planes=2):
    groups = FEED_HEAD_GROUPS if groups is None else groups
    if planes == 3:
        return 0
    return int(_lib.load().pgasr_gemm_x3w_feed_head_items(int(N), int(K), int(groups))) if groups > 0 else 0


def gemm_x3w_feed(A, planes, C, M, N, K, bias, busy_ptr, tiles_done, order=0, phase=0, ws=None, ctrl=None):
    lib = _lib.load()
    for t, nm in ((A, "A"), (C, "C"), (bias, "bias")):
        if t is not None and (not t.is_cuda or t.dtype != torch.float32):
            raise _lib.PgasrError(f"gemm_x3w_feed operand {nm} must be a float32 GPU tensor")
    _check_planes(planes, N, K, "gemm_x3w_feed")
    if tiles_done.dtype != torch.int32 or tiles_done.numel() < 2 * ((M + 255) // 256):
        raise _lib.PgasrError("gemm_x3w_feed: tiles_done must hold 2 * ceil(M/256) int32 words")
    if len(planes) == 3:
        if phase == 2 and ws is None:
            raise _lib.PgasrError("gemm_x3w_feed: phase 2 continues the queue of a phase-1 call: pass its workspace")
        if ws is None:
            ws = _workspace(lib.pgasr_gemm_x6w_feed_workspace_bytes(), C.device, "x6w_feed")
        with _timed("gemm_feed_x6c"):
            if ctrl is not None and (ctrl.dtype != torch.int32 or ctrl.numel() < 256 or not ctrl.is_contiguous()):
                raise _lib.PgasrError("gemm_x3w_feed: ctrl = 256 zeroed int32 words")
            st = lib.pgasr_gemm_x6w_feed_phase_f32(M, N, K, A.data_ptr(), K, *_plane_ptrs(planes), C.data_ptr(), N, _p(bias),
                                                   busy_ptr, tiles_done.data_ptr(), int(order), int(phase), _p(ctrl), _p(ws), ws.numel(), _stream())
        _lib.check(st, "pgasr_gemm_x6w_feed_phase_f32")
        return ws if phase == 1 else C
    if ws is None:
        ws = _workspace(lib.pgasr_gemm_x3w_feed_workspace_bytes(), C.device, "x3w_feed")
    with _timed("gemm_feed_x3w"):
        st = lib.pgasr_gemm_x3w_feed_f32(M, N, K, A.data_ptr(), K, planes[0].data_ptr(), planes[1].data_ptr(), C.data_ptr(), N, _p(bias),
                                         busy_ptr, tiles_done.data_ptr(), int(order), int(phase), FEED_HEAD_GROUPS if phase else 0,
                                         _p(ws), ws.numel(), _stream())
    _lib.check(st, "pgasr_gemm_x3w_feed_f32")
    return ws if phase == 1 else C


def lstm_layer_bwd(gates, out, cbuf, dout, pack_b, lengths, T, B, want_dbias=False, fed=None, fed_need=0, drop=None, slab=None):
    lib = _lib.load()
    ws = _lstm_ws(T, B, True, gates.device)
    part = torch.empty((B + 15) // 16, 2 * 4 * HID, dtype=torch.float32, device=gates.device) if want_dbias else None
    with _timed("lstm_bwd_kernel"):
        if slab is not None:
            words = slab
            if words.dtype != torch.int32 or not words.is_cuda or words.numel() < 2 * ((B + 15) // 16):
                raise _lib.PgasrError("lstm_layer_bwd: slab_done must be an int32 GPU tensor of 2 * ceil(B/16) words")
            p, seed, offset = drop if drop is not None else (0.0, 0, 0)
            st = lib.pgasr_lstm_layer_bwd_streamed(_p(gates), _p(out), _p(cbuf), _p(dout), _p(pack_b), _p(lengths), T, B, _lstm_flags(pack_b),
                                                   _p(part), _p(fed), int(fed_need), float(p), int(seed), int(offset),
                                                   _p(words), _p(ws), ws.numel(), _stream())
        elif fed is None:
            st = lib.pgasr_lstm_layer_bwd(_p(gates), _p(out), _p(cbuf), _p(dout), _p(pack_b), _p(lengths), T, B, _lstm_flags(pack_b),
# ... 273 lines not shown
```

### policy_gradient_asr_amd/model.py

```python
import torch
import torch.nn as nn

from . import functional as Fh
from . import hipops
from . import streams

HID = 256


def weights(m):
    if isinstance(m, nn.Linear):
        nn.init.xavier_normal_(m.weight.data)
        nn.init.constant_(m.bias.data, 0.1)


def nan_to_num(t, mynan=0.):
    if torch.all(torch.isfinite(t)):
        return t
    return torch.where(torch.isfinite(t), t, torch.as_tensor(mynan, dtype=t.dtype, device=t.device))


class Encoder(nn.Module):

    def __init__(self, n_feats=120):
        super().__init__()
        self.n_feats = n_feats
        self.inst_norm = nn.InstanceNorm2d(n_feats)
        self.input_layer = nn.Linear(n_feats, 512)
        self.blstm = nn.LSTM(input_size=512, hidden_size=HID, num_layers=3, dropout=0.3,
                             bidirectional=True, batch_first=True)
        self.drop = nn.Dropout()
        self.dropout_seed = 0x5EED
        self._drop_calls = 0

    def _layer_params(self, l):
        out = []
        for sfx in ("", "_reverse"):
            for k in ("weight_ih", "weight_hh", "bias_ih", "bias_hh"):
                out.append(getattr(self.blstm, f"{k}_l{l}{sfx}"))
        return out

    def forward_time_major(self, x, mask, lengths=None):
        if not x.is_cuda:
            raise RuntimeError("policy_gradient_asr_amd.Encoder runs on the MI355X only (no CPU fallback)")
        if lengths is None:
            lengths = mask.sum(dim=1).to(torch.int32).contiguous()
        training = self.training
        packs = Fh.prepack_blstm_layers([self._layer_params(l) for l in range(3)], [512, 512, 512],
                                        rows=x.shape[0] * x.shape[2])
        y = Fh.InstNormAffineFn.apply(x.float(), self.input_layer.weight, self.input_layer.bias, True)
        h = y
        if training:
            h = Fh.DropoutFn.apply(h, self.drop.p, self.dropout_seed, self._next_drop_offset(), True)
        for l in range(3):
            od = (self.blstm.dropout, self.dropout_seed, self._next_drop_offset()) if (training and l < 2 and self.blstm.dropout > 0) else None
            h = Fh.blstm_layer(h, lengths, self._layer_params(l), dact_y=y if (l == 0 and not training) else None,
                               sweep_follows=(l > 0), prepacked=packs[l], out_dropout=od)
        return h, lengths

    def _next_drop_offset(self):
        self._drop_calls += 1
        return self._drop_calls

    def forward(self, x, mask):
        h, _ = self.forward_time_major(x, mask)
        return h.transpose(0, 1)


class Attention(nn.Module):

    def __init__(self):
        super().__init__()

    def forward(self, dec_t, enc_out):
        from . import hipops
        return hipops.attention_ctx(dec_t.contiguous(), enc_out.contiguous())


class Decoder(nn.Module):

    def __init__(self, alphabet_size, hidden_size):
        super().__init__()
        self.alphabet_size = alphabet_size
        self.hidden_size = hidden_size
        self.embed_layer = nn.Embedding(alphabet_size, 128)
        self.lstm = nn.LSTM(input_size=128, hidden_size=hidden_size, num_layers=1, batch_first=True)
        self.attn = Attention()

    def forward(self, target_inputs, encoder_outputs, device=None):
        from . import hipops
        H = self.hidden_size
        w_ih, w_hh = self.lstm.weight_ih_l0.detach().contiguous(), self.lstm.weight_hh_l0.detach().contiguous()
        bias = (self.lstm.bias_ih_l0 + self.lstm.bias_hh_l0).detach().contiguous()
        if not w_ih.is_cuda:
            raise RuntimeError("Decoder.forward runs on the MI355X only (no CPU path)")
        B, L = target_inputs.shape
        x = self.embed_layer.weight.detach()[target_inputs.to(w_ih.device)].transpose(0, 1).contiguous()
        xp = torch.empty(L * B, 4 * H, dtype=torch.float32, device=w_ih.device)
        hipops.gemm(x.view(L * B, 128), w_ih, xp, M=L * B, N=4 * H, K=128, transB=True, bias=bias, precision=0)
        xp = xp.view(L, B, 4 * H)
        h = torch.zeros(B, H, dtype=torch.float32, device=w_ih.device)
        c = torch.zeros_like(h)
        g = torch.empty(B, 4 * H, dtype=torch.float32, device=w_ih.device)
        dec_out = torch.empty(L, B, H, dtype=torch.float32, device=w_ih.device)
        for t in range(L):
            hipops.gemm(h, w_hh, g, M=B, N=4 * H, K=H, transB=True, precision=0)
            hipops.lstm_cell(g, xp[t], c, h, dec_out[t])
        ctx = hipops.attention_ctx(dec_out, encoder_outputs.to(w_ih.device).contiguous())
        return torch.cat((dec_out, ctx), dim=2)


class Seq2Seq(nn.Module):

    def __init__(self, alphabet_size, n_feats=120):
        super().__init__()
        self.encoder = Encoder(n_feats=n_feats)
        self.head = nn.Linear(2 * HID, alphabet_size)

    def logits(self, x, fmask, lengths=None):
        h, lengths = self.encoder.forward_time_major(x, fmask, lengths)
        if hipops.head_logsoftmax_ok(self.head.in_features, self.head.out_features):
            z, lp = Fh.HeadFn.apply(h, self.head.weight, self.head.bias)
            z.log_probs = lp
            z.log_probs_version = z._version
            return z, lengths
        return Fh.LinearFn.apply(h, self.head.weight, self.head.bias), lengths

    def forward(self, x, t, fmask, device=None):
        z, _ = self.logits(x, fmask)
        return Fh.LogSoftmaxFn.apply(z)


def _read_alphabet(alphabet_path):
    with open(alphabet_path, "r") as fo:
        alphabet = ["<pad>"] + fo.readlines()
    char2ind = {alphabet[i].replace("\n", ""): i for i in range(len(alphabet))}
    return alphabet, char2ind


def _to_device(batch, device):
    x = batch["feat"].to(device)
    t = batch["trans"].to(device)
    fmask = batch["fmask"].squeeze(1).to(device)
    tmask = batch["tmask"].squeeze(1).to(device)
    return x, t, fmask, tmask


FEATURE_DIMS = {"mfcc": 120, "logmel80": 80}


def _check_features(features, n_feats, dataset):
    if features not in FEATURE_DIMS:
        raise ValueError(f"features must be one of {sorted(FEATURE_DIMS)}")
    try:
        item = dataset[0] if dataset is not None and len(dataset) > 0 else None
    except Exception:
        item = None
    if isinstance(item, dict) and ("wave" in item or "aud" in item) and "feat" not in item:
        if n_feats != FEATURE_DIMS[features]:
            raise ValueError(f"features='{features}' gives {FEATURE_DIMS[features]} features per frame but n_feats={n_feats}")


def train(corpus_path, model_path, num_epochs, batch_size, device, train_dataset=None, dev_dataset=None,
          n_feats=120, lam=1.0, lr=5e-4, resume=True, log_every=10, seed=0, bucket_by_length=True, features="mfcc",
          precision="f32", num_samples=1, reward_baseline="hypothesis", reward_unit="char", max_grad_norm=None):
    import os
    import numpy as np
    import torch.utils.data as tud
    import functools
    from .data import Data, LengthBucketSampler, dataset_lengths
    from .data import collate_custom as _collate
    from .loss import pg_ctc_loss
    from .train_step import PolicyGradientTrainer

    print("Num epochs:", num_epochs, "Batch size:", batch_size)
    alphabet_path = os.path.join(corpus_path, "alphabet.txt")
    alphabet, char2ind = _read_alphabet(alphabet_path)
    word_delimiter = None
    if reward_unit == "word":
        if " " not in char2ind:
            raise ValueError(f"reward_unit='word' splits words at the alphabet's ' ' symbol, and {alphabet_path} has none")
        word_delimiter = char2ind[" "]
    dev = torch.device("cuda", device if isinstance(device, int) else 0) if not isinstance(device, torch.device) else device
    os.makedirs(model_path, exist_ok=True)
    collate_custom = functools.partial(_collate, device=dev, features=features)
    if train_dataset is None:
        train_dataset = Data(os.path.join(corpus_path, "train.tsv"), os.path.join(corpus_path, "clips"), char2ind)
    if dev_dataset is None and os.path.exists(os.path.join(corpus_path, "dev.tsv")):
        dev_dataset = Data(os.path.join(corpus_path, "dev.tsv"), os.path.join(corpus_path, "clips"), char2ind)

    torch.manual_seed(seed)
    model = Seq2Seq(alphabet_size=len(char2ind), n_feats=n_feats)
    model.apply(weights)
    model = model.to(dev)
    _check_features(features, n_feats, train_dataset)
    trainer = PolicyGradientTrainer(model, lr=lr, lam=lam, seed=seed, precision=precision, num_samples=num_samples,
                                    reward_baseline=reward_baseline, reward_unit=reward_unit, word_delimiter=word_delimiter,
                                    max_grad_norm=max_grad_norm)
    losses, val_losses, best, start_epoch = [], [], 9999999.0, 1
    ckpt = os.path.join(model_path, "checkpoint_last.pth")
    if resume and os.path.exists(ckpt):
        st = torch.load(ckpt, map_location=dev)
        model.load_state_dict(st["model"])
        from .train_step import FLAG_PAD
        trainer.exp_avg[FLAG_PAD:].copy_(st["exp_avg"]); trainer.exp_avg_sq[FLAG_PAD:].copy_(st["exp_avg_sq"]); trainer.nstep = st["nstep"]
        trainer.set_applied_steps(st.get("applied_steps", st["nstep"]))
# ... 112 lines not shown
```

Measured before the change: 3320.

## Fuse input dropout into affine GEMM epilogue and add skinny weight-grad kernels

Applies the training dropout mask inside the input-affine GEMM's store epilogue, using Philox keyed by element index, so the separate dropout kernel and its extra read and write of the activation go away. Adds a dedicated skinny weight-gradient kernel for the output head (V<=128) and for the input affine layer, which folds the leaky-ReLU derivative and dropout mask recomputation into the dW/db reduction instead of running a general split-K GEMM plus a colsum. This brings extra code paths and relies on recomputing the mask bit-identically in backward. The dropout epilogue is limited to the exact-fp32 path.

Result: no change. 3341, median of 6 (+0.6%).

```diff
diff --git a/include/pgasr_hip.h b/include/pgasr_hip.h
--- a/include/pgasr_hip.h
+++ b/include/pgasr_hip.h
@@ -100,6 +100,13 @@
                    const float* bias, const float* bias2, int act, float slope, int accumulate,
                    const float* dact_y, int norm_operand, const float* shift, const float* scale,
                    int precision, const unsigned* xcc_busy, void* workspace, size_t workspace_bytes, void* stream);
+int pgasr_gemm_f32_dropout(int transA, int transB, int M, int N, int K, float alpha,
+                           const float* A, int lda, long long strideA,
+                           const float* B, int ldb, long long strideB,
+                           float* C, int ldc, long long strideC, int batch,
+                           const float* bias, const float* bias2, int act, float slope,
+                           int norm_operand, const float* shift, const float* scale,
+                           float drop_p, uint64_t drop_seed, uint32_t drop_offset, void* stream);
 
 int pgasr_split_bf16_planes(const float* src, int rows, int cols, int ld, int transpose,
                             unsigned short* hi, unsigned short* lo, void* stream);
@@ -145,6 +152,14 @@
 size_t pgasr_colsum_workspace_bytes(int rows, int cols);
 int pgasr_colsum_f32(const float* X, int rows, int cols, int ld, float* out, float* out2, int accumulate,
                      void* workspace, size_t workspace_bytes, void* stream);
+
+size_t pgasr_head_wgrad_workspace_bytes(long long rows, int V, int N);
+int pgasr_head_wgrad_f32(const float* dlogits, const float* x, long long rows, int V, int N, float* dW, float* db,
+                         int accumulate, void* workspace, size_t workspace_bytes, void* stream);
+size_t pgasr_affine_wgrad_workspace_bytes(int B, int F, int T, int N);
+int pgasr_affine_wgrad_f32(const float* x, const float* shift, const float* scale, const float* dx, const float* act_y,
+                           float slope, float p, uint64_t seed, uint32_t offset, int B, int F, int T, int N,
+                           float* dW, float* db, int accumulate, void* workspace, size_t workspace_bytes, void* stream);
 
 int pgasr_instnorm_stats(const float* x, int B, int F, int T, float eps, float* mean, float* rstd,
                          void* stream);
diff --git a/policy_gradient_asr_amd/_lib.py b/policy_gradient_asr_amd/_lib.py
--- a/policy_gradient_asr_amd/_lib.py
+++ b/policy_gradient_asr_amd/_lib.py
@@ -61,6 +61,11 @@
                                  c_f32p, C.c_int, C.c_longlong, C.c_int, C.c_int, C.c_int,
                                  c_f32p, c_f32p, C.c_int, C.c_float, C.c_int,
                                  c_f32p, C.c_int, c_f32p, c_f32p, C.c_int, c_ptr, c_ptr, C.c_size_t, c_ptr]),
+    "pgasr_gemm_f32_dropout": (C.c_int, [C.c_int, C.c_int, C.c_int, C.c_int, C.c_int, C.c_float,
+                                         c_f32p, C.c_int, C.c_longlong, c_f32p, C.c_int, C.c_longlong,
+                                         c_f32p, C.c_int, C.c_longlong, C.c_int,
+                                         c_f32p, c_f32p, C.c_int, C.c_float,
+                                         C.c_int, c_f32p, c_f32p, C.c_float, C.c_uint64, C.c_uint32, c_ptr]),
     "pgasr_split_bf16_planes": (C.c_int, [c_f32p, C.c_int, C.c_int, C.c_int, C.c_int, c_ptr, c_ptr, c_ptr]),
     "pgasr_gemm_x3w_f32": (C.c_int, [C.c_int, C.c_int, C.c_int, c_f32p, C.c_int, c_ptr, c_ptr, c_f32p, C.c_int,
                                      c_f32p, c_f32p, C.c_float, c_ptr]),
@@ -77,6 +82,12 @@
     "pgasr_colsum_workspace_bytes": (C.c_size_t, [C.c_int, C.c_int]),
     "pgasr_colsum_f32": (C.c_int, [c_f32p, C.c_int, C.c_int, C.c_int, c_f32p, c_f32p, C.c_int,
                                    c_ptr, C.c_size_t, c_ptr]),
+    "pgasr_head_wgrad_workspace_bytes": (C.c_size_t, [C.c_longlong, C.c_int, C.c_int]),
+    "pgasr_head_wgrad_f32": (C.c_int, [c_f32p, c_f32p, C.c_longlong, C.c_int, C.c_int, c_f32p, c_f32p, C.c_int,
+                                       c_ptr, C.c_size_t, c_ptr]),
+    "pgasr_affine_wgrad_workspace_bytes": (C.c_size_t, [C.c_int, C.c_int, C.c_int, C.c_int]),
+    "pgasr_affine_wgrad_f32": (C.c_int, [c_f32p, c_f32p, c_f32p, c_f32p, c_f32p, C.c_float, C.c_float, C.c_uint64, C.c_uint32,
+                                         C.c_int, C.c_int, C.c_int, C.c_int, c_f32p, c_f32p, C.c_int, c_ptr, C.c_size_t, c_ptr]),
     "pgasr_instnorm_stats": (C.c_int, [c_f32p, C.c_int, C.c_int, C.c_int, C.c_float, c_f32p, c_f32p, c_ptr]),
     "pgasr_log_softmax_rows": (C.c_int, [c_f32p, C.c_longlong, C.c_int, c_f32p, c_ptr]),
     "pgasr_lstm_pack_bytes": (C.c_size_t, [C.c_int, C.c_int]),
diff --git a/policy_gradient_asr_amd/csrc/common.h b/policy_gradient_asr_amd/csrc/common.h
--- a/policy_gradient_asr_amd/csrc/common.h
+++ b/policy_gradient_asr_amd/csrc/common.h
@@ -56,6 +56,14 @@
     out[0] = c0; out[1] = c1; out[2] = c2; out[3] = c3;
 }
 
+__device__ __forceinline__ void keep4(unsigned long long quad, uint32_t offset, uint32_t k0, uint32_t k1,
+                                      uint32_t thresh, bool keep[4]) {
+    uint32_t r[4];
+    philox4x32_10((uint32_t)quad, (uint32_t)(quad >> 32), offset, 0u, k0, k1, r);
+#pragma unroll
+    for (int i = 0; i < 4; ++i) keep[i] = r[i] >= thresh;
+}
+
 #ifndef PGASR_WSLAB_NUM
 #define PGASR_WSLAB_NUM 5
 #define PGASR_WSLAB_DEN 4
diff --git a/policy_gradient_asr_amd/csrc/gemm.hip b/policy_gradient_asr_amd/csrc/gemm.hip
--- a/policy_gradient_asr_amd/csrc/gemm.hip
+++ b/policy_gradient_asr_amd/csrc/gemm.hip
@@ -24,6 +24,8 @@
     const unsigned* xcc_busy;
     int tx, ty, tz;
     int wide;
+    int drop;
+    uint32_t drop_thresh, drop_k0, drop_k1, drop_off; float drop_scale;
 };
 
 __device__ __forceinline__ void store_tiles_fast(const GemmArgs& g, const f32x16 (&acc)[2][2], int m0, int n0, int wm, int wn,
@@ -100,6 +102,50 @@
                 v = (lk && !(v > 0.f)) ? v * g.slope : v;
                 v = v * f[r] + c0[r];
                 __builtin_amdgcn_raw_buffer_store_b32(__float_as_uint(v), crs, o, 0, 0);
+            }
+        }
+}
+
+__device__ __forceinline__ void store_tiles_drop(const GemmArgs& g, const f32x16 (&acc)[2][2], int m0, int n0, int wm, int wn,
+                                                 int lane, int bidx) {
+    const int cl = lane & 31, rq = lane >> 5, w = lane & 3;
+    float* Cb = g.C + (size_t)bidx * g.sC;
+    const unsigned cbytes = (unsigned)(((size_t)(g.M - 1) * g.ldc + g.N) * 4);
+    __amdgpu_buffer_rsrc_t crs = __builtin_amdgcn_make_buffer_rsrc(Cb, 0, (int)cbytes, 0x00020000);
+    const bool lk = g.act == 1;
+#pragma unroll
+    for (int i = 0; i < 2; ++i)
+#pragma unroll
+        for (int j = 0; j < 2; ++j) {
+            const int n = n0 + wn * 64 + j * 32 + cl;
+            const bool ok = n < g.N;
+            float bsum = 0.f;
+            if (ok) {
+                if (g.bias) bsum += g.bias[n];
+                if (g.bias2) bsum += g.bias2[n];
+            }
+            const int mrow = m0 + wm * 64 + i * 32 + 4 * rq;
+            unsigned keepbits = 0;
+#pragma unroll
+            for (int q = 0; q < 4; ++q) {
+                const unsigned long long idx = (unsigned long long)bidx * g.sC + (unsigned long long)(mrow + w + 8 * q) * g.ldc + (n & ~3);
+                uint32_t rnd[4];
+                philox4x32_10((uint32_t)(idx >> 2), (uint32_t)(idx >> 34), g.drop_off, 0u, g.drop_k0, g.drop_k1, rnd);
+#pragma unroll
+                for (int d = 0; d < 4; ++d) {
+                    const int k = w ^ d;
+                    const uint32_t mine = k == 0 ? rnd[0] : k == 1 ? rnd[1] : k == 2 ? rnd[2] : rnd[3];
+                    const uint32_t got = (uint32_t)__shfl_xor((int)mine, d, 64);
+                    keepbits |= (got >= g.drop_thresh ? 1u : 0u) << (k + 4 * q);
+                }
+            }
+            const unsigned o0 = (unsigned)(((size_t)mrow * g.ldc + n) * 4);
+#pragma unroll
+            for (int r = 0; r < 16; ++r) {
+                float v = g.alpha * acc[i][j][r] + bsum;
+                v = (lk && !(v > 0.f)) ? v * g.slope : v;
+                v = ((keepbits >> r) & 1u) ? v * g.drop_scale : 0.f;
+                __builtin_amdgcn_raw_buffer_store_b32(__float_as_uint(v), crs, ok ? o0 + (unsigned)(((r & 3) + 8 * (r >> 2)) * g.ldc * 4) : 0xFFFFFFFFu, 0, 0);
             }
         }
 }
@@ -244,6 +290,7 @@
         cur ^= 1;
     }
 
+    if (g.drop) { store_tiles_drop(g, acc, m0, n0, wm, wn, lane, bidx); return; }
     if (!g.wide) { store_tiles_fast(g, acc, m0, n0, wm, wn, lane, z, bidx, true); return; }
     const int cl = lane & 31, rq = lane >> 5;
 #pragma unroll
@@ -675,14 +722,15 @@
     return 256 + (size_t)batch * splitk * M * N * sizeof(float);
 }
 
-extern "C" int pgasr_gemm_f32(int transA, int transB, int M, int N, int K, float alpha,
-                              const float* A, int lda, long long strideA,
-                              const float* B, int ldb, long long strideB,
-                              float* C, int ldc, long long strideC,
-                              int batch, int sum_batches, int splitk,
-                              const float* bias, const float* bias2, int act, float slope, int accumulate,
-                              const float* dact_y, int norm_operand, const float* shift, const float* scale,
-                              int precision, const unsigned* xcc_busy, void* workspace, size_t workspace_bytes, void* stream) {
+static int gemm_f32_entry(int transA, int transB, int M, int N, int K, float alpha,
+                          const float* A, int lda, long long strideA,
+                          const float* B, int ldb, long long strideB,
+                          float* C, int ldc, long long strideC,
+                          int batch, int sum_batches, int splitk,
+                          const float* bias, const float* bias2, int act, float slope, int accumulate,
+                          const float* dact_y, int norm_operand, const float* shift, const float* scale,
+                          int precision, const unsigned* xcc_busy, void* workspace, size_t workspace_bytes, void* stream,
+                          bool drop, float drop_p, uint64_t drop_seed, uint32_t drop_offset) {
     if (!A || !B || !C || M <= 0 || N <= 0 || K <= 0 || batch <= 0 || splitk <= 0) return PGASR_ERR_INVALID_ARG;
     if (norm_operand < 0 || norm_operand > 2 || (norm_operand && (!shift || !scale))) return PGASR_ERR_INVALID_ARG;
     if (act < 0 || act > 1 || precision < 0 || precision > 2) return PGASR_ERR_INVALID_ARG;
@@ -697,7 +745,42 @@
     g.alpha = alpha; g.bias = bias; g.bias2 = bias2; g.act = act; g.slope = slope; g.accumulate = accumulate;
     g.dact_y = dact_y; g.norm_operand = norm_operand; g.shift = shift; g.scale = scale; g.partial = nullptr;
     g.wide = (((size_t)(M - 1) * ldc + N) * 4 >= ((size_t)1 << 32) || (size_t)M * N * 4 >= ((size_t)1 << 32)) ? 1 : 0;
+    g.drop = 0; g.drop_thresh = g.drop_k0 = g.drop_k1 = g.drop_off = 0; g.drop_scale = 1.f;
+    if (drop) {
+        if (!(drop_p >= 0.f) || !(drop_p < 1.f)) return PGASR_ERR_INVALID_ARG;
+        if (precision != 0 || splitk != 1 || sum_batches || accumulate || dact_y || g.wide || (ldc & 3) || (strideC & 3) || strideC < 0)
+            return PGASR_ERR_UNSUPPORTED;
+        g.drop = 1;
+        g.drop_thresh = (uint32_t)fmin(4294967295.0, (double)drop_p * 4294967296.0);
+        g.drop_scale = 1.f / (1.f - drop_p);
+        g.drop_k0 = (uint32_t)(drop_seed & 0xffffffffu); g.drop_k1 = (uint32_t)(drop_seed >> 32); g.drop_off = drop_offset;
+    }
     return gemm_launch(g, transA, transB, sum_batches, precision, xcc_busy, workspace, workspace_bytes, (hipStream_t)stream);
+}
+
+extern "C" int pgasr_gemm_f32(int transA, int transB, int M, int N, int K, float alpha,
+                              const float* A, int lda, long long strideA,
+                              const float* B, int ldb, long long strideB,
+                              float* C, int ldc, long long strideC,
+                              int batch, int sum_batches, int splitk,
+                              const float* bias, const float* bias2, int act, float slope, int accumulate,
+                              const float* dact_y, int norm_operand, const float* shift, const float* scale,
+                              int precision, const unsigned* xcc_busy, void* workspace, size_t workspace_bytes, void* stream) {
+    return gemm_f32_entry(transA, transB, M, N, K, alpha, A, lda, strideA, B, ldb, strideB, C, ldc, strideC, batch, sum_batches, splitk,
+                          bias, bias2, act, slope, accumulate, dact_y, norm_operand, shift, scale, precision, xcc_busy, workspace,
+                          workspace_bytes, stream, false, 0.f, 0, 0);
+}
+
+extern "C" int pgasr_gemm_f32_dropout(int transA, int transB, int M, int N, int K, float alpha,
+                                      const float* A, int lda, long long strideA,
+                                      const float* B, int ldb, long long strideB,
+                                      float* C, int ldc, long long strideC, int batch,
+                                      const float* bias, const float* bias2, int act, float slope,
+                                      int norm_operand, const float* shift, const float* scale,
+                                      float drop_p, uint64_t drop_seed, uint32_t drop_offset, void* stream) {
+    return gemm_f32_entry(transA, transB, M, N, K, alpha, A, lda, strideA, B, ldb, strideB, C, ldc, strideC, batch, 0, 1,
+                          bias, bias2, act, slope, 0, nullptr, norm_operand, shift, scale, 0, nullptr, nullptr, 0, stream,
+                          true, drop_p, drop_seed, drop_offset);
 }
 
 extern "C" int pgasr_lstm_wgrad_slabs(int T, int* edges, int max_edges) {
diff --git a/policy_gradient_asr_amd/csrc/optim.hip b/policy_gradient_asr_amd/csrc/optim.hip
--- a/policy_gradient_asr_amd/csrc/optim.hip
+++ b/policy_gradient_asr_amd/csrc/optim.hip
@@ -1,14 +1,6 @@
 #include "common.h"
 
 namespace {
-
-__device__ __forceinline__ void keep4(unsigned long long quad, uint32_t offset, uint32_t k0, uint32_t k1,
-                                      uint32_t thresh, bool keep[4]) {
-    uint32_t r[4];
-    philox4x32_10((uint32_t)quad, (uint32_t)(quad >> 32), offset, 0u, k0, k1, r);
-#pragma unroll
-    for (int i = 0; i < 4; ++i) keep[i] = r[i] >= thresh;
-}
 
 __global__ __launch_bounds__(256) void dropout_kernel(const float* __restrict__ x, float* __restrict__ y,
                                                       unsigned long long n, uint32_t thresh, float scale,
diff --git a/policy_gradient_asr_amd/csrc/skinny.hip b/policy_gradient_asr_amd/csrc/skinny.hip
--- /dev/null
+++ b/policy_gradient_asr_amd/csrc/skinny.hip
@@ -0,0 +1,298 @@
+#include "common.h"
+
+namespace {
+
+typedef __attribute__((ext_vector_type(16))) float f32x16;
+
+constexpr int SK_CH = 128;
+constexpr int SK_PF = 16;
+constexpr int SK_BIAS_PITCH = 128;
+constexpr int SK_GROUP = 16;
+
+struct SkinnyArgs {
+    const float* v;
+    const float* sgn;
+    const float* u;
+    const float* shift; const float* scale;
+    float* partial;
+    float* biasp;
+    int mode, S, Stot, N;
+    int B; long long T;
+    int nbl;
+    int bgroups;
+    float slope, dscale;
+    uint32_t thresh, k0, k1, offset; int drop;
+};
+
+template <int ST, bool SGN, bool DROP, bool VBIAS>
+__global__ __launch_bounds__(256) void skinny_wgrad_kernel(SkinnyArgs a) {
+    constexpr int SP = 32 * ST, NSTEP = SK_CH / 2;
+    __shared__ float us[SK_CH * SP];
+    const int tid = threadIdx.x, lane = tid & 63, wave = tid >> 6;
+    const int j = lane & 31, kk = lane >> 5;
+    const int chunk = blockIdx.x;
+    const int b0 = (chunk % a.bgroups) << a.nbl;
+    const long long t0 = (long long)(chunk / a.bgroups) * (SK_CH >> a.nbl);
+    const int nbm = (1 << a.nbl) - 1;
+    const int ncol = blockIdx.y * 512 + wave * 128 + 4 * j;
+    const bool wave_live = blockIdx.y * 512 + wave * 128 < a.N;
+
+    auto row_off = [&](int i) -> long long {
+        const long long t = t0 + (i >> a.nbl);
+        const int b = b0 + (i & nbm);
+        return (wave_live && t < a.T && b < a.B) ? (t * a.B + b) * (long long)a.N + ncol : -1;
+    };
+    auto issue = [&](int step, float4& v, float4& s) {
+        const long long off = row_off(2 * step + kk);
+        const float4 lv = *reinterpret_cast<const float4*>(a.v + (off < 0 ? 0 : off));
+        v = off < 0 ? make_float4(0.f, 0.f, 0.f, 0.f) : lv;
+        if constexpr (SGN) s = *reinterpret_cast<const float4*>(a.sgn + (off < 0 ? 0 : off));
+    };
+    float4 vb[SK_PF], sb[SK_PF];
+#pragma unroll
+    for (int k = 0; k < SK_PF; ++k) issue(k, vb[k], sb[k]);
+
+    if (a.mode == 0) {
+#pragma unroll 8
+        for (int idx = tid; idx < SK_CH * SP; idx += 256) {
+            const int i = idx / SP, s = idx % SP;
+            const long long r = t0 + i;
+            const bool ok = r < a.T && s < a.S;
+            const float val = a.u[ok ? r * a.S + s : 0];
+            us[idx] = ok ? val : 0.f;
+        }
+    } else if ((a.T & 3) == 0 && (((size_t)a.u) & 15) == 0) {
+        const int nql = 5 - a.nbl, nqm = (SK_CH >> (a.nbl + 2)) - 1;
+#pragma unroll 4
+        for (int idx = tid; idx < SK_CH * SP / 4; idx += 256) {
+            const int tq = idx & nqm, q = idx >> nql;
+            const int f = q % SP, bb = q / SP;
+            const long long t = t0 + 4 * tq;
+            const int b = b0 + bb;
+            const bool row = t < a.T && b < a.B, ok = row && f < a.S;
+            const int bc = row ? b : 0;
+            const float4 xv = *reinterpret_cast<const float4*>(a.u + (ok ? ((long long)b * a.S + f) * a.T + t : 0));
+            const float sh = a.shift[bc], sc = a.scale[bc];
+            float* dst = us + (((4 * tq) << a.nbl) + bb) * SP + f;
+            const int rp = SP << a.nbl;
+            dst[0] = ok ? (xv.x - sh) * sc : 0.f; dst[rp] = ok ? (xv.y - sh) * sc : 0.f;
+            dst[2 * rp] = ok ? (xv.z - sh) * sc : 0.f; dst[3 * rp] = ok ? (xv.w - sh) * sc : 0.f;
+        }
+    } else {
+        const int ntl = 7 - a.nbl, ntm = (SK_CH >> a.nbl) - 1;
+#pragma unroll 8
+        for (int idx = tid; idx < SK_CH * SP; idx += 256) {
+            const int tt = idx & ntm, q = idx >> ntl;
+            const int f = q % SP, bb = q / SP;
+            const long long t = t0 + tt;
+            const int b = b0 + bb;
+            const bool row = t < a.T && b < a.B, ok = row && f < a.S;
+            const int bc = row ? b : 0;
+            const float val = (a.u[ok ? ((long long)b * a.S + f) * a.T + t : 0] - a.shift[bc]) * a.scale[bc];
+            us[((tt << a.nbl) + bb) * SP + f] = ok ? val : 0.f;
+        }
+    }
+    __syncthreads();
+    if (a.mode == 0 && blockIdx.y == 0 && tid < a.S) {
+        float s[4] = {0.f, 0.f, 0.f, 0.f};
+        for (int i = 0; i < SK_CH; i += 4) {
+#pragma unroll
+            for (int k = 0; k < 4; ++k) s[k] += us[(i + k) * SP + tid];
+        }
+        a.biasp[(size_t)chunk * SK_BIAS_PITCH + tid] = (s[0] + s[1]) + (s[2] + s[3]);
+    }
+    float4 bsum[2] = {make_float4(0.f, 0.f, 0.f, 0.f), make_float4(0.f, 0.f, 0.f, 0.f)};
+
+    f32x16 acc[ST][4];
+#pragma unroll
+    for (int st = 0; st < ST; ++st)
+#pragma unroll
+        for (int c = 0; c < 4; ++c)
+#pragma unroll
+            for (int r = 0; r < 16; ++r) acc[st][c][r] = 0.f;
+
+    for (int s0 = 0; s0 < NSTEP; s0 += SK_PF) {
+#pragma unroll
+        for (int k = 0; k < SK_PF; ++k) {
+            const int step = s0 + k;
+            float4 v = vb[k];
+            if constexpr (SGN) {
+                const float4 s = sb[k];
+                v.x *= s.x > 0.f ? 1.f : a.slope; v.y *= s.y > 0.f ? 1.f : a.slope;
+                v.z *= s.z > 0.f ? 1.f : a.slope; v.w *= s.w > 0.f ? 1.f : a.slope;
+            }
+            if constexpr (DROP) {
+                const long long off = row_off(2 * step + kk);
+                bool keep[4];
+                keep4((unsigned long long)(off < 0 ? 0 : off) >> 2, a.offset, a.k0, a.k1, a.thresh, keep);
+                v.x = keep[0] ? v.x * a.dscale : 0.f; v.y = keep[1] ? v.y * a.dscale : 0.f;
+                v.z = keep[2] ? v.z * a.dscale : 0.f; v.w = keep[3] ? v.w * a.dscale : 0.f;
+            }
+            if constexpr (VBIAS) {
+                float4& bs = bsum[k & 1];
+                bs.x += v.x; bs.y += v.y; bs.z += v.z; bs.w += v.w;
+            }
+            if (step + SK_PF < NSTEP) issue(step + SK_PF, vb[k], sb[k]);
+            float au[ST];
+#pragma unroll
+            for (int st = 0; st < ST; ++st) au[st] = us[(2 * step + kk) * SP + st * 32 + j];
+#pragma unroll
+            for (int st = 0; st < ST; ++st) {
+                acc[st][0] = __builtin_amdgcn_mfma_f32_32x32x2f32(au[st], v.x, acc[st][0], 0, 0, 0);
+                acc[st][1] = __builtin_amdgcn_mfma_f32_32x32x2f32(au[st], v.y, acc[st][1], 0, 0, 0);
+                acc[st][2] = __builtin_amdgcn_mfma_f32_32x32x2f32(au[st], v.z, acc[st][2], 0, 0, 0);
+                acc[st][3] = __builtin_amdgcn_mfma_f32_32x32x2f32(au[st], v.w, acc[st][3], 0, 0, 0);
+            }
+        }
+    }
+
+    if (!wave_live) return;
+    if constexpr (VBIAS) {
+        float4 t[2];
+#pragma unroll
+        for (int p = 0; p < 2; ++p) {
+            t[p].x = bsum[p].x + __shfl_xor(bsum[p].x, 32, 64); t[p].y = bsum[p].y + __shfl_xor(bsum[p].y, 32, 64);
+            t[p].z = bsum[p].z + __shfl_xor(bsum[p].z, 32, 64); t[p].w = bsum[p].w + __shfl_xor(bsum[p].w, 32, 64);
+        }
+        if (kk == 0)
+            *reinterpret_cast<float4*>(a.biasp + (size_t)chunk * a.N + ncol) =
+                make_float4(t[0].x + t[1].x, t[0].y + t[1].y, t[0].z + t[1].z, t[0].w + t[1].w);
+    }
+    float* slab = a.partial + (size_t)chunk * a.Stot * a.N + ncol;
+#pragma unroll
+    for (int st = 0; st < ST; ++st)
+#pragma unroll
+        for (int r = 0; r < 16; ++r) {
+            const int s = st * 32 + (r & 3) + 8 * (r >> 2) + 4 * kk;
+            if (s < a.Stot)
+                *reinterpret_cast<float4*>(slab + (size_t)s * a.N) = make_float4(acc[st][0][r], acc[st][1][r], acc[st][2][r], acc[st][3][r]);
+        }
+}
+
+__device__ __forceinline__ float skinny_grouped_sum(const float* __restrict__ p, size_t stride, int n) {
+    float v = 0.f;
+    int c = 0;
+    for (; c + SK_GROUP <= n; c += SK_GROUP) {
+        float t[SK_GROUP];
+#pragma unroll
+        for (int i = 0; i < SK_GROUP; ++i) t[i] = p[(size_t)(c + i) * stride];
+        float g = 0.f;
+#pragma unroll
+        for (int i = 0; i < SK_GROUP; ++i) g += t[i];
+        v += g;
+    }
+    if (c < n) {
+        float g = 0.f;
+        for (; c < n; ++c) g += p[(size_t)c * stride];
+        v += g;
+    }
+    return v;
+}
+
+__global__ __launch_bounds__(64) void skinny_reduce_kernel(const float* __restrict__ partial, const float* __restrict__ biasp,
+                                                           int nchunks, int S, int N, int mode,
+                                                           float* __restrict__ dW, float* __restrict__ db, int accumulate) {
+    const size_t idx = (size_t)blockIdx.x * 64 + threadIdx.x;
+    const size_t slab = (size_t)S * N;
+    const size_t nbias = mode == 0 ? (size_t)S : (size_t)N;
+    float v;
+    float* out;
+    if (idx < slab) {
+        v = skinny_grouped_sum(partial + idx, slab, nchunks);
+        const int s = (int)(idx / N), n = (int)(idx % N);
+        out = mode == 0 ? dW + idx : dW + (size_t)n * S + s;
+    } else if (idx < slab + nbias) {
+        const size_t k = idx - slab;
+        v = skinny_grouped_sum(biasp + k, mode == 0 ? (size_t)SK_BIAS_PITCH : (size_t)N, nchunks);
+        out = db + k;
+    } else {
+        return;
+    }
+    *out = accumulate ? *out + v : v;
+}
+
+struct SkinnyPlan { int nbl, bgroups; long long chunks; int Stot, ST; size_t partial_bytes, bytes; };
+
+bool skinny_plan(int mode, long long T, int B, int S, int N, SkinnyPlan& p) {
+    if (T <= 0 || B <= 0 || S <= 0 || N <= 0 || (N & 127)) return false;
+    p.Stot = S;
+    if (S > 128) return false;
+    p.ST = (p.Stot + 31) / 32;
+    p.nbl = 0;
+    if (mode == 1) while (p.nbl < 3 && (2 << p.nbl) <= B) ++p.nbl;
+    const int NB = 1 << p.nbl, NT = SK_CH >> p.nbl;
+    p.bgroups = (B + NB - 1) / NB;
+    p.chunks = (long long)p.bgroups * ((T + NT - 1) / NT);
+    if (p.chunks > 0x7fffffffLL || T * B >= ((long long)1 << 40)) return false;
+    p.partial_bytes = (size_t)p.chunks * p.Stot * N * sizeof(float);
+    p.bytes = p.partial_bytes + (size_t)p.chunks * (mode == 0 ? SK_BIAS_PITCH : N) * sizeof(float);
+    return true;
+}
+
+int skinny_launch(SkinnyArgs a, const SkinnyPlan& p, float* dW, float* db, int accumulate, void* workspace, size_t workspace_bytes,
+                  hipStream_t st) {
+    if (!workspace || workspace_bytes < p.bytes) return PGASR_ERR_WORKSPACE;
+    if ((((size_t)a.v) | ((size_t)a.sgn) | ((size_t)workspace)) & 15) return PGASR_ERR_INVALID_ARG;
+    a.partial = (float*)workspace;
+    a.biasp = (float*)((char*)workspace + p.partial_bytes);
+    a.Stot = p.Stot; a.nbl = p.nbl; a.bgroups = p.bgroups;
+    const dim3 grid((unsigned)p.chunks, (unsigned)((a.N + 511) / 512));
+#define SK_LAUNCH(ST_) do { \
+        if (a.mode == 0) PGASR_LAUNCH_KERNEL((skinny_wgrad_kernel<ST_, false, false, false>), grid, dim3(256), 0, st, a); \
+        else if (a.sgn && a.drop) PGASR_LAUNCH_KERNEL((skinny_wgrad_kernel<ST_, true, true, true>), grid, dim3(256), 0, st, a); \
+        else if (a.sgn) PGASR_LAUNCH_KERNEL((skinny_wgrad_kernel<ST_, true, false, true>), grid, dim3(256), 0, st, a); \
+        else if (a.drop) PGASR_LAUNCH_KERNEL((skinny_wgrad_kernel<ST_, false, true, true>), grid, dim3(256), 0, st, a); \
+        else PGASR_LAUNCH_KERNEL((skinny_wgrad_kernel<ST_, false, false, true>), grid, dim3(256), 0, st, a); } while (0)
+    switch (p.ST) {
+        case 1: SK_LAUNCH(1); break;
+        case 2: SK_LAUNCH(2); break;
+        case 3: SK_LAUNCH(3); break;
+        default: SK_LAUNCH(4); break;
+    }
+#undef SK_LAUNCH
+    PGASR_CHECK_LAUNCH();
+    const size_t outs = (size_t)a.S * a.N + (a.mode == 0 ? a.S : a.N);
+    PGASR_LAUNCH_KERNEL(skinny_reduce_kernel, dim3((unsigned)((outs + 63) / 64)), dim3(64), 0, st, a.partial, a.biasp,
+                       (int)p.chunks, a.S, a.N, a.mode, dW, db, accumulate);
+    PGASR_CHECK_LAUNCH();
+    return PGASR_OK;
+}
+
+}
+
+extern "C" size_t pgasr_head_wgrad_workspace_bytes(long long rows, int V, int N) {
+    SkinnyPlan p;
+    return skinny_plan(0, rows, 1, V, N, p) ? p.bytes : 0;
+}
+
+extern "C" int pgasr_head_wgrad_f32(const float* dlogits, const float* x, long long rows, int V, int N, float* dW, float* db,
+                                    int accumulate, void* workspace, size_t workspace_bytes, void* stream) {
+    if (!dlogits || !x || !dW || !db || rows <= 0 || V <= 0 || N <= 0) return PGASR_ERR_INVALID_ARG;
+    SkinnyPlan p;
+    if (!skinny_plan(0, rows, 1, V, N, p)) return PGASR_ERR_UNSUPPORTED;
+    SkinnyArgs a{};
+    a.v = x; a.u = dlogits; a.mode = 0; a.S = V; a.N = N; a.B = 1; a.T = rows;
+    return skinny_launch(a, p, dW, db, accumulate, workspace, workspace_bytes, (hipStream_t)stream);
+}
+
+extern "C" size_t pgasr_affine_wgrad_workspace_bytes(int B, int F, int T, int N) {
+    SkinnyPlan p;
+    return skinny_plan(1, T, B, F, N, p) ? p.bytes : 0;
+}
+
+extern "C" int pgasr_affine_wgrad_f32(const float* x, const float* shift, const float* scale, const float* dx, const float* act_y,
+                                      float slope, float p_drop, uint64_t seed, uint32_t offset, int B, int F, int T, int N,
+                                      float* dW, float* db, int accumulate, void* workspace, size_t workspace_bytes, void* stream) {
+    if (!x || !shift || !scale || !dx || !dW || !db || B <= 0 || F <= 0 || T <= 0 || N <= 0) return PGASR_ERR_INVALID_ARG;
+    if (!(p_drop >= 0.f) || !(p_drop < 1.f)) return PGASR_ERR_INVALID_ARG;
+    SkinnyPlan p;
+    if (!skinny_plan(1, T, B, F, N, p)) return PGASR_ERR_UNSUPPORTED;
+    SkinnyArgs a{};
+    a.v = dx; a.sgn = act_y; a.u = x; a.shift = shift; a.scale = scale; a.mode = 1; a.S = F; a.N = N; a.B = B; a.T = T;
+    a.slope = slope;
+    a.drop = p_drop > 0.f ? 1 : 0;
+    a.thresh = (uint32_t)fmin(4294967295.0, (double)p_drop * 4294967296.0);
+    a.dscale = 1.f / (1.f - p_drop);
+    a.k0 = (uint32_t)(seed & 0xffffffffu); a.k1 = (uint32_t)(seed >> 32); a.offset = offset;
+    return skinny_launch(a, p, dW, db, accumulate, workspace, workspace_bytes, (hipStream_t)stream);
+}
diff --git a/policy_gradient_asr_amd/functional.py b/policy_gradient_asr_amd/functional.py
--- a/policy_gradient_asr_amd/functional.py
+++ b/policy_gradient_asr_amd/functional.py
@@ -131,16 +131,22 @@
 class InstNormAffineFn(torch.autograd.Function):
 
     @staticmethod
-    def forward(ctx, x, weight, bias, consumer_applies_dact=False):
+    def forward(ctx, x, weight, bias, consumer_applies_dact=False, drop=None):
         B, F, T = x.shape
         N = weight.shape[0]
         x = x.contiguous(); weight = weight.contiguous(); bias = bias.contiguous()
         ctx.consumer_applies_dact = bool(consumer_applies_dact)
+        ctx.drop = (float(drop[0]), int(drop[1]), int(drop[2])) if drop is not None else None
+        if ctx.drop is not None and ctx.consumer_applies_dact:
+            raise ValueError("InstNormAffineFn: with drop the backward applies leaky' itself")
         mean, rstd = hipops.instnorm_stats(x, 1e-5)
         y = torch.empty(T, B, N, dtype=torch.float32, device=x.device)
+        fused_drop = ctx.drop if (ctx.drop is not None and hipops.affine_dropout_ok(B, T, N)) else None
         hipops.gemm(x, weight, y, M=T, N=N, K=F, transA=True, transB=True, lda=T, ldb=F, ldc=B * N,
                     strideA=F * T, strideB=0, strideC=N, batch=B, bias=bias, act=1, slope=LEAKY_SLOPE,
-                    norm_operand=1, shift=mean, scale=rstd, precision=0)
+                    norm_operand=1, shift=mean, scale=rstd, precision=0, drop=fused_drop)
+        if ctx.drop is not None and fused_drop is None:
+            hipops.dropout(y, *ctx.drop, out=y)
         ctx.save_for_backward(x, weight, mean, rstd, y)
         ctx.bias_ref, ctx.weight_ref = bias, weight
         return y
@@ -150,13 +156,23 @@
         x, weight, mean, rstd, y = ctx.saved_tensors
         B, F, T = x.shape
         N = weight.shape[0]
-        if ctx.consumer_applies_dact:
-            dpre = dy.contiguous()
+        dy = dy.contiguous()
+        act_y = None if ctx.consumer_applies_dact else y
+        wg, bg = getattr(ctx.weight_ref, "grad", None), getattr(ctx.bias_ref, "grad", None)
+        direct = (grad_overlap.enabled and wg is not None and bg is not None and wg.is_contiguous() and bg.is_contiguous()
+                  and wg.dtype == torch.float32 and bg.dtype == torch.float32 and tuple(wg.shape) == (N, F))
+        if hipops.affine_wgrad_ok(B, F, T, N):
+            dW = wg if direct else torch.empty(N, F, dtype=torch.float32, device=x.device)
+            db = bg if direct else torch.empty(N, dtype=torch.float32, device=x.device)
+            hipops.affine_wgrad(x, mean, rstd, dy, dW, db, act_y=act_y, slope=LEAKY_SLOPE, drop=ctx.drop, accumulate=direct)
+            return (None, None, None, None, None) if direct else (None, dW, db, None, None)
+        if ctx.drop is not None:
+            dpre = hipops.dropout(dy, *ctx.drop, dact_y=act_y, slope=LEAKY_SLOPE)
+        elif act_y is not None:
+            dpre = torch.where(y > 0, dy, dy * LEAKY_SLOPE).contiguous()
         else:
-            dpre = torch.where(y > 0, dy, dy * LEAKY_SLOPE).contiguous()
-        bg = getattr(ctx.bias_ref, "grad", None)
-        if grad_overlap.enabled and bg is not None and bg.is_contiguous() and bg.dtype == torch.float32:
-            main = torch.cuda.current_stream()
+            dpre = dy
+        if direct:
             side = grad_overlap.side_stream()
             ready = torch.cuda.Event()
             ready.record()
@@ -164,14 +180,11 @@
                 side.wait_event(ready)
                 hipops.colsum(dpre, T * B, N, N, bg, accumulate=True)
             streams.hold(dpre, side)
-            wg = getattr(ctx.weight_ref, "grad", None)
-            direct = wg is not None and wg.is_contiguous() and wg.dtype == torch.float32 and tuple(wg.shape) == (N, F)
-            dW = wg if direct else torch.empty(N, F, dtype=torch.float32, device=x.device)
-            hipops.gemm(dpre, x, dW, M=N, N=F, K=T, transA=True, transB=True, lda=B * N, ldb=T, ldc=F,
+            hipops.gemm(dpre, x, wg, M=N, N=F, K=T, transA=True, transB=True, lda=B * N, ldb=T, ldc=F,
                         strideA=N, strideB=F * T, strideC=0, batch=B, sum_batches=True, norm_operand=2,
-                        shift=mean, scale=rstd, accumulate=direct, splitk=AFFINE_DW_SPLITK if T >= 256 else 1)
-            return (None, None if direct else dW, None, None)
-        return (None, *InstNormAffineFn.param_grads(x, mean, rstd, dpre, N), None)
+                        shift=mean, scale=rstd, accumulate=True, splitk=AFFINE_DW_SPLITK if T >= 256 else 1)
+            return (None, None, None, None, None)
+        return (None, *InstNormAffineFn.param_grads(x, mean, rstd, dpre, N), None, None)
 
     @staticmethod
     def param_grads(x, mean, rstd, dpre, N):
@@ -233,12 +246,16 @@
         dx = torch.empty(rows, K, dtype=torch.float32, device=dy.device)
         hipops.gemm(dy2, weight, dx, M=rows, N=K, K=N)
         wg, bg = (p.grad for p in ctx.param_refs)
+        skinny = hipops.head_wgrad_ok(rows, N, K)
         if grad_overlap.enabled and wg is not None and bg is not None and wg.is_contiguous() and bg.is_contiguous():
             done = torch.cuda.Event()
             done.record()
             grad_overlap.note_event(done)
 
             def weight_grads():
+                if skinny:
+                    hipops.head_wgrad(dy2, x2, wg, bg, accumulate=True)
+                    return
                 hipops.gemm(dy2, x2, wg, M=N, N=K, K=rows, transA=True, lda=N, splitk=_pick_splitk(N, K, rows), accumulate=True)
                 hipops.colsum(dy2, rows, N, N, bg, accumulate=True)
             grad_overlap.pending().append((done, weight_grads))
@@ -246,8 +263,11 @@
             streams.hold(dy2, side); streams.hold(x2, side)
             return dx.view(ctx.shp), None, None
         dW = torch.empty(N, K, dtype=torch.float32, device=dy.device)
+        db = torch.empty(N, dtype=torch.float32, device=dy.device)
+        if skinny:
+            hipops.head_wgrad(dy2, x2, dW, db)
+            return dx.view(ctx.shp), dW, db
         hipops.gemm(dy2, x2, dW, M=N, N=K, K=rows, transA=True, lda=N, splitk=_pick_splitk(N, K, rows))
-        db = torch.empty(N, dtype=torch.float32, device=dy.device)
         hipops.colsum(dy2, rows, N, N, db)
         return dx.view(ctx.shp), dW, db
 
diff --git a/policy_gradient_asr_amd/hipops.py b/policy_gradient_asr_amd/hipops.py
--- a/policy_gradient_asr_amd/hipops.py
+++ b/policy_gradient_asr_amd/hipops.py
@@ -444,10 +444,12 @@
 def gemm(A, B, C, M, N, K, transA=False, transB=False, lda=None, ldb=None, ldc=None, alpha=1.0,
          strideA=0, strideB=0, strideC=0, batch=1, sum_batches=False, splitk=1, bias=None, bias2=None,
          act=0, slope=0.01, accumulate=False, dact_y=None, norm_operand=0, shift=None, scale=None,
-         a_off=0, b_off=0, c_off=0, precision=None, xcc_busy=None):
+         a_off=0, b_off=0, c_off=0, precision=None, xcc_busy=None, drop=None):
     lib = _lib.load()
     if precision is None:
         precision = GEMM_PRECISION
+    if drop is not None and (precision != 0 or sum_batches or splitk != 1 or accumulate or dact_y is not None or xcc_busy is not None):
+        raise _lib.PgasrError("gemm: the dropout epilogue exists for the plain exact-fp32 product only")
     for t, nm in ((A, "A"), (B, "B"), (C, "C"), (bias, "bias"), (bias2, "bias2"), (dact_y, "dact_y"),
                   (shift, "shift"), (scale, "scale")):
         if t is not None:
@@ -456,6 +458,15 @@
     lda = lda if lda is not None else (M if transA else K)
     ldb = ldb if ldb is not None else (K if transB else N)
     ldc = ldc if ldc is not None else N
+    if drop is not None:
+        with _timed("gemm_f32"):
+            st = lib.pgasr_gemm_f32_dropout(int(transA), int(transB), M, N, K, float(alpha),
+                                            A.data_ptr() + 4 * a_off, lda, int(strideA), B.data_ptr() + 4 * b_off, ldb, int(strideB),
+                                            C.data_ptr() + 4 * c_off, ldc, int(strideC), batch, _p(bias), _p(bias2), act, float(slope),
+                                            norm_operand, _p(shift), _p(scale), float(drop[0]), int(drop[1]) & (2 ** 64 - 1),
+                                            int(drop[2]) & 0xFFFFFFFF, _stream())
+        _lib.check(st, "pgasr_gemm_f32_dropout")
+        return C
     nbytes = lib.pgasr_gemm_workspace_bytes(M, N, batch, splitk, int(sum_batches))
     ws = _workspace(nbytes, C.device, "gemm")
     with _timed("gemm_f32"):
@@ -557,6 +568,48 @@
     st = lib.pgasr_colsum_f32(_p(X), rows, cols, ld, _p(out), _p(out2), int(accumulate), _p(ws), ws.numel(), _stream())
     _lib.check(st, "pgasr_colsum_f32")
     return out
+
+
+def head_wgrad_ok(rows, V, N):
+    return rows > 0 and 0 < V <= 128 and N > 0 and N % 128 == 0
+
+
+def head_wgrad(dlogits, x, dW, db, accumulate=False):
+    lib = _lib.load()
+    for t, nm in ((dlogits, "dlogits"), (x, "x"), (dW, "dW"), (db, "db")):
+        _req(t, torch.float32, nm)
+    rows, V = dlogits.shape
+    N = x.shape[1]
+    if x.shape[0] != rows or tuple(dW.shape) != (V, N) or db.numel() != V:
+        raise _lib.PgasrError("head_wgrad: shapes do not match")
+    ws = _workspace(lib.pgasr_head_wgrad_workspace_bytes(rows, V, N), x.device, "skinny")
+    with _timed("head_wgrad"):
+        st = lib.pgasr_head_wgrad_f32(_p(dlogits), _p(x), rows, V, N, _p(dW), _p(db), int(accumulate), _p(ws), ws.numel(), _stream())
+    _lib.check(st, "pgasr_head_wgrad_f32")
+
+
+def affine_dropout_ok(B, T, N):
+    return N % 4 == 0 and T * B * N * 4 < 2 ** 32
+
+
+def affine_wgrad_ok(B, F, T, N):
+    return B > 0 and T > 0 and 0 < F <= 128 and N > 0 and N % 128 == 0
+
+
+def affine_wgrad(x, mean, rstd, dx, dW, db, act_y=None, slope=0.01, drop=None, accumulate=False):
+    lib = _lib.load()
+    for t, nm in ((x, "x"), (mean, "mean"), (rstd, "rstd"), (dx, "dx"), (dW, "dW"), (db, "db"), (act_y, "act_y")):
+        _req(t, torch.float32, nm)
+    B, F, T = x.shape
+    N = dx.shape[-1]
+    if dx.numel() != T * B * N or tuple(dW.shape) != (N, F) or db.numel() != N or (act_y is not None and act_y.numel() != dx.numel()):
+        raise _lib.PgasrError("affine_wgrad: shapes do not match")
+    p, seed, offset = drop if drop is not None else (0.0, 0, 0)
+    ws = _workspace(lib.pgasr_affine_wgrad_workspace_bytes(B, F, T, N), x.device, "skinny")
+    with _timed("affine_wgrad"):
+        st = lib.pgasr_affine_wgrad_f32(_p(x), _p(mean), _p(rstd), _p(dx), _p(act_y), float(slope), float(p), int(seed) & (2 ** 64 - 1),
+                                        int(offset) & 0xFFFFFFFF, B, F, T, N, _p(dW), _p(db), int(accumulate), _p(ws), ws.numel(), _stream())
+    _lib.check(st, "pgasr_affine_wgrad_f32")
 
 
 def instnorm_stats(x, eps=1e-5):
diff --git a/policy_gradient_asr_amd/model.py b/policy_gradient_asr_amd/model.py
--- a/policy_gradient_asr_amd/model.py
+++ b/policy_gradient_asr_amd/model.py
@@ -48,10 +48,9 @@
         training = self.training
         packs = Fh.prepack_blstm_layers([self._layer_params(l) for l in range(3)], [512, 512, 512],
                                         rows=x.shape[0] * x.shape[2])
-        y = Fh.InstNormAffineFn.apply(x.float(), self.input_layer.weight, self.input_layer.bias, True)
+        drop = (self.drop.p, self.dropout_seed, self._next_drop_offset()) if training else None
+        y = Fh.InstNormAffineFn.apply(x.float(), self.input_layer.weight, self.input_layer.bias, not training, drop)
         h = y
-        if training:
-            h = Fh.DropoutFn.apply(h, self.drop.p, self.dropout_seed, self._next_drop_offset(), True)
         for l in range(3):
             od = (self.blstm.dropout, self.dropout_seed, self._next_drop_offset()) if (training and l < 2 and self.blstm.dropout > 0) else None
             h = Fh.blstm_layer(h, lengths, self._layer_params(l), dact_y=y if (l == 0 and not training) else None,
```
